# Bostanabad-Research-Group/GP-Plus

Hardware: AMD Instinct MI355X
Metric: MLL evals/sec (fwd+grad), NxN exact GP, N=20k d=8 (higher is better)
Workload: dtype f64; 1 GPU; C2: synthetic Borehole (Sobol seed 0, unique rows, z-scored) N=20000 d=8 fp64, GP_Plus Rough_RBF exact GP at theta1, one replica per GPU (restart-parallel); N=20000, d=8, streams_per_gpu=1

## Files before the change

gp-plus_amd/_lib.py:

```python
from __future__ import annotations

import ctypes
import os
import subprocess
from ctypes import POINTER, c_char_p, c_double, c_int, c_int32, c_int64, c_size_t, c_void_p
from pathlib import Path

import torch

_PKG_DIR = Path(__file__).resolve().parent
_LIB_PATH = _PKG_DIR / "libgpp_hip.so"
_CSRC = _PKG_DIR / "csrc"

_SIGNATURES = {
    "gpp_version": (c_char_p, []),
    "gpp_create": (c_int, [POINTER(c_void_p), c_int]),
    "gpp_destroy": (c_int, [c_void_p]),
    "gpp_set_stream": (c_int, [c_void_p, c_void_p]),
    "gpp_internal_stream": (c_int, [c_void_p, c_int, POINTER(c_void_p)]),
    "gpp_set_option": (c_int, [c_void_p, c_int, c_int]),
    "gpp_workspace_bytes": (c_size_t, [c_void_p, c_int, c_int64, c_int64, c_int, c_int]),
    "gpp_set_workspace": (c_int, [c_void_p, c_void_p, c_size_t]),
    "gpp_kernel_build": (c_int, [c_void_p, c_void_p, c_int64, c_int, c_void_p, c_void_p, c_void_p, c_void_p, c_int,
                                 c_double, c_int, c_int, c_int, c_void_p, c_int64, c_int64, c_int64]),
    "gpp_cross_kernel": (c_int, [c_void_p, c_void_p, c_int64, c_void_p, c_int64, c_int, c_void_p, c_void_p, c_int,
                                 c_int, c_void_p, c_int64]),
    "gpp_kernel_apply": (c_int, [c_void_p, c_void_p, c_int64, c_void_p, c_int64, c_int, c_void_p, c_void_p, c_int, c_int, c_void_p,
                                 c_int64, c_int, c_double, c_void_p, c_int64]),
    "gpp_rff_apply": (c_int, [c_void_p, c_void_p, c_int64, c_int, c_void_p, c_void_p, c_int64, c_void_p, c_void_p, c_int64, c_int,
                              c_double, c_void_p, c_int64]),
    "gpp_kernel_apply_grad": (c_int, [c_void_p, c_void_p, c_int64, c_void_p, c_int64, c_int, c_void_p, c_void_p, c_int, c_int, c_void_p,
                                      c_int64, c_int, c_void_p, c_int64, c_double, c_void_p, c_int64]),
    "gpp_rff_apply_grad": (c_int, [c_void_p, c_void_p, c_int64, c_int, c_void_p, c_void_p, c_int64, c_void_p, c_void_p, c_int64, c_int,
                                   c_void_p, c_int64, c_double, c_void_p, c_int64]),
    "gpp_potrf": (c_int, [c_void_p, c_void_p, c_int64, c_int64, c_void_p, c_int64, c_void_p]),
    "gpp_potrf_ws": (c_int, [c_void_p, c_void_p, c_int64, c_int64, c_void_p, c_int64, c_void_p, c_int64, c_void_p]),
    "gpp_build_potrf_ws": (c_int, [c_void_p, c_void_p, c_int64, c_int, c_void_p, c_void_p, c_void_p, c_void_p, c_int, c_double, c_int,
                                   c_int, c_void_p, c_int64, c_void_p, c_int64, c_void_p, c_int64, c_void_p]),
    "gpp_trtri": (c_int, [c_void_p, c_void_p, c_int64, c_int64, c_void_p, c_int64, c_void_p, c_int64]),
    "gpp_lauum": (c_int, [c_void_p, c_void_p, c_int64, c_int64, c_void_p, c_int64]),
    "gpp_lauum_grad": (c_int, [c_void_p, c_void_p, c_int64, c_int64, c_void_p, c_int, c_void_p, c_void_p, c_void_p, c_int, c_int, c_int,
                               c_void_p, c_void_p, c_void_p, c_void_p]),
    "gpp_post_cov_train": (c_int, [c_void_p, c_void_p, c_int64, c_int64, c_void_p, c_void_p, c_int, c_void_p, c_double, c_void_p,
                                   c_int64]),
    "gpp_syrk_rows": (c_int, [c_void_p, c_void_p, c_int64, c_void_p, c_int64, c_int64, c_int64, c_int64, c_int64, c_int, c_int]),
    "gpp_gemm_lower_cols": (c_int, [c_void_p, c_void_p, c_int64, c_void_p, c_int64, c_void_p, c_int64, c_int64, c_int64, c_double,
                                    c_double, c_int64, c_int64, c_int, c_int, c_int64, c_int64, c_int]),
    "gpp_shard_list_begin": (c_int, [c_void_p, c_int64, c_int64, c_int, c_int, c_void_p, c_int64, c_void_p, c_void_p, c_int64, c_void_p,
                                     c_void_p, c_void_p, c_void_p, c_int64, c_void_p, c_int, POINTER(c_int)]),
    "gpp_shard_piece_cols": (c_int64, []),
    "gpp_shard_list_gate": (c_int, [c_void_p, c_void_p, c_int, c_int]),
    "gpp_shard_list_signal": (c_int, [c_void_p, c_void_p, c_int, c_int]),
    "gpp_shard_list_end": (c_int, [c_void_p]),
    "gpp_set_comm": (c_int, [c_void_p, c_void_p, c_int, c_int]),
    "gpp_comm_unique_id": (c_int, [c_void_p]),
    "gpp_comm_init_rccl": (c_int, [c_void_p, c_void_p, c_int, c_int]),
    "gpp_shard_buffer_doubles": (c_size_t, [c_int64, c_int64, c_int, c_int, c_int]),
    "gpp_shard_eval": (c_int, [c_void_p, c_int64, c_int64, c_void_p, c_int, c_void_p, c_void_p, c_void_p, c_void_p, c_int, c_int, c_int,
                               c_double, c_int, c_int, c_void_p, POINTER(c_int)]),
    "gpp_push_create": (c_int, [c_int, c_int, c_int, c_int64, POINTER(c_void_p), c_void_p]),
    "gpp_push_connect": (c_int, [c_void_p, c_void_p]),
    "gpp_push_send": (c_int, [c_void_p, c_void_p, c_int64, c_void_p, c_int, c_int, POINTER(c_void_p), POINTER(c_int64), POINTER(c_int64),
                              POINTER(c_int64), POINTER(c_int64), POINTER(c_int64)]),
    "gpp_push_recv": (c_int, [c_void_p, c_void_p, c_int64, c_void_p, c_int, c_int, POINTER(c_void_p), POINTER(c_int64), POINTER(c_int64),
                              POINTER(c_int64), POINTER(c_int64), POINTER(c_int64)]),
    "gpp_push_ack": (c_int, [c_void_p, c_void_p, c_int64]),
    "gpp_push_info": (c_int, [c_void_p, POINTER(c_int64), POINTER(c_int)]),
    "gpp_push_destroy": (c_int, [c_void_p, c_int]),
    "gpp_shard_back_list": (c_int, [c_void_p, c_int64, c_int64, c_int, c_int, c_void_p, c_int64, c_void_p, c_void_p, c_int64, c_void_p,
                                    c_void_p, c_int, POINTER(c_int)]),
    "gpp_trmv_lower_cols": (c_int, [c_void_p, c_void_p, c_int64, c_int64, c_void_p, c_void_p, c_int64, c_int, c_int, c_int, c_int]),
    "gpp_mll_scalars": (c_int, [c_void_p, c_void_p, c_int64, c_int64, c_void_p, c_void_p]),
    "gpp_grad_reduce_cols": (c_int, [c_void_p, c_void_p, c_int64, c_int, c_void_p, c_void_p, c_void_p, c_int, c_int, c_int,
                                     c_void_p, c_void_p, c_int64, c_int, c_int64, c_int, c_int, c_void_p, c_void_p, c_void_p,
                                     c_void_p, c_int]),
    "gpp_lauum_rows": (c_int, [c_void_p, c_void_p, c_int64, c_int64, c_void_p, c_int64, c_int, c_int]),
    "gpp_lauum_rows_range": (c_int, [c_void_p, c_void_p, c_int64, c_int64, c_void_p, c_int64, c_int, c_int, c_int64, c_int64]),
    "gpp_transpose": (c_int, [c_void_p, c_void_p, c_int64, c_int64, c_int64, c_void_p, c_int64]),
    "gpp_mll_reduce": (c_int, [c_void_p, c_void_p, c_int64, c_void_p, c_int64, c_int64, c_void_p, c_void_p, c_void_p]),
    "gpp_alpha": (c_int, [c_void_p, c_void_p, c_int64, c_int64, c_void_p, c_void_p]),
    "gpp_grad_reduce": (c_int, [c_void_p, c_void_p, c_int64, c_int, c_void_p, c_void_p, c_void_p, c_int, c_int, c_int,
                                c_void_p, c_void_p, c_int64, c_int, c_void_p, c_void_p, c_void_p, c_void_p]),
    "gpp_loo_scalars": (c_int, [c_void_p, c_void_p, c_int64, c_int64, c_void_p, c_void_p, c_void_p, c_void_p, c_void_p, c_void_p, c_void_p,
                                c_void_p]),
    "gpp_sym_rowscale": (c_int, [c_void_p, c_void_p, c_int64, c_int64, c_void_p, c_void_p, c_int64]),
    "gpp_loo_grad_reduce": (c_int, [c_void_p, c_void_p, c_int64, c_int, c_void_p, c_void_p, c_void_p, c_int, c_int, c_int,
                                    c_void_p, c_void_p, c_void_p, c_int64, c_int, c_void_p, c_void_p, c_void_p, c_void_p]),
    "gpp_grad_reduce_rows": (c_int, [c_void_p, c_void_p, c_int64, c_int, c_void_p, c_void_p, c_void_p, c_int, c_int, c_int,
                                     c_void_p, c_void_p, c_int64, c_int, c_int64, c_int, c_int, c_void_p, c_void_p, c_void_p,
                                     c_void_p]),
    "gpp_predict": (c_int, [c_void_p, c_void_p, c_int64, c_int64, c_void_p, c_void_p, c_int64, c_int64, c_void_p,
                            c_void_p, c_int64, c_void_p, c_void_p]),
    "gpp_predict_tn": (c_int, [c_void_p, c_void_p, c_int64, c_int64, c_void_p, c_void_p, c_int64, c_int64, c_void_p,
                               c_void_p, c_int64, c_void_p, c_void_p]),
    "gpp_cross_grad": (c_int, [c_void_p, c_void_p, c_int64, c_void_p, c_int64, c_int, c_void_p, c_void_p, c_int, c_int, c_void_p,
                               c_void_p, c_void_p, c_void_p, c_int64, c_void_p, c_int, c_void_p, c_int, c_void_p, c_void_p]),
    "gpp_gemm": (c_int, [c_void_p, c_int, c_int, c_int64, c_int64, c_int64, c_double, c_void_p, c_int64, c_void_p,
                         c_int64, c_double, c_void_p, c_int64, c_int, c_int, c_int, c_int, c_int]),
    "gpp_gemm_batched": (c_int, [c_void_p, c_int, c_int, c_int64, c_int64, c_int64, c_double, c_void_p, c_int64, c_int64,
                                 c_void_p, c_int64, c_int64, c_double, c_void_p, c_int64, c_int64, c_int, c_int, c_int, c_int,
                                 c_int, c_int]),
    "gpp_kernel_build_batched": (c_int, [c_void_p, c_void_p, c_int64, c_int64, c_int, c_void_p, c_void_p, c_void_p, c_void_p, c_int,
                                         c_double, c_int, c_int, c_int, c_void_p, c_int64, c_int64, c_int]),
    "gpp_potrf_batched": (c_int, [c_void_p, c_void_p, c_int64, c_int64, c_int64, c_void_p, c_int64, c_int64, c_void_p, c_int]),
    "gpp_trtri_batched": (c_int, [c_void_p, c_void_p, c_int64, c_int64, c_int64, c_void_p, c_int64, c_int64, c_void_p, c_int64,
                                  c_int64, c_int]),
    "gpp_lauum_batched": (c_int, [c_void_p, c_void_p, c_int64, c_int64, c_int64, c_void_p, c_int64, c_int64, c_int]),
    "gpp_mll_reduce_batched": (c_int, [c_void_p, c_void_p, c_int64, c_int64, c_void_p, c_int64, c_int64, c_int64, c_void_p,
                                       c_void_p, c_int64, c_void_p, c_int]),
    "gpp_alpha_batched": (c_int, [c_void_p, c_void_p, c_int64, c_int64, c_int64, c_void_p, c_void_p, c_int64, c_int]),
    "gpp_grad_reduce_batched": (c_int, [c_void_p, c_void_p, c_int64, c_int64, c_int, c_void_p, c_void_p, c_void_p, c_int, c_int,
                                        c_int, c_void_p, c_int64, c_void_p, c_int64, c_int64, c_int, c_void_p, c_void_p, c_void_p,
                                        c_void_p, c_int]),
    "gpp_loo_scalars_batched": (c_int, [c_void_p, c_void_p, c_int64, c_int64, c_int64, c_void_p, c_void_p, c_void_p, c_void_p, c_void_p,
                                        c_void_p, c_void_p, c_int64, c_void_p, c_int]),
    "gpp_sym_rowscale_batched": (c_int, [c_void_p, c_void_p, c_int64, c_int64, c_int64, c_void_p, c_int64, c_void_p, c_int64, c_int64,
                                         c_int]),
    "gpp_loo_grad_reduce_batched": (c_int, [c_void_p, c_void_p, c_int64, c_int64, c_int, c_void_p, c_void_p, c_void_p, c_int, c_int,
                                            c_int, c_void_p, c_void_p, c_int64, c_void_p, c_int64, c_int64, c_int, c_void_p, c_void_p,
                                            c_void_p, c_void_p, c_int]),
    "gpp_cv_blocks": (c_int, [c_void_p, c_void_p, c_int64, c_int64, c_void_p, c_void_p, c_int, c_int, c_void_p, c_int64, c_int64]),
    "gpp_cv_rows": (c_int, [c_void_p, c_void_p, c_int64, c_int64, c_void_p, c_void_p, c_int, c_void_p, c_int64, c_int64, c_void_p,
                            c_int64]),
    "gpp_chol_append": (c_int, [c_void_p, c_void_p, c_int64, c_void_p, c_int64, c_int64, c_int64, c_void_p, c_int64, c_void_p, c_int64,
                                c_void_p, c_void_p, c_void_p, c_void_p]),
    "gpp_post_cross_sq": (c_int, [c_void_p, c_void_p, c_int64, c_void_p, c_int64, c_int, c_void_p, c_void_p, c_int, c_int, c_void_p,
                                  c_int64, c_void_p, c_int64, c_int64, c_int, c_void_p, c_void_p]),
    "gpp_post_cross_min": (c_int, [c_void_p, c_void_p, c_int64, c_void_p, c_int64, c_int, c_void_p, c_void_p, c_int, c_int, c_void_p,
                                   c_int64, c_void_p, c_int64, c_int64, c_int, c_void_p, c_void_p, c_void_p, c_int, c_void_p]),
    "gpp_cross_kernel_dx": (c_int, [c_void_p, c_void_p, c_int64, c_void_p, c_int64, c_int, c_void_p, c_void_p, c_int, c_int, c_int,
                                    c_int, c_void_p, c_int64]),
    "gpp_point_gram": (c_int, [c_void_p, c_void_p, c_int64, c_int64, c_int, c_int64, c_void_p, c_void_p, c_void_p]),
    "gpp_kernel_dxdx": (c_int, [c_void_p, c_void_p, c_int64, c_void_p, c_int64, c_int, c_void_p, c_void_p, c_int, c_int, c_int,
                                c_int, c_void_p, c_int64]),
}

_lib = None


class GppError(RuntimeError):
    """A libgpp_hip call returned a non-zero status."""


def build(force: bool = False) -> Path:
    if force:
        subprocess.run(["make", "-C", str(_CSRC), "clean"], check=True, capture_output=True)
    proc = subprocess.run(["make", "-C", str(_CSRC), "-j4"], capture_output=True, text=True)
    if proc.returncode != 0:
        raise RuntimeError("building libgpp_hip.so failed:\n" + proc.stdout + proc.stderr)
    return _LIB_PATH


def load() -> ctypes.CDLL:
    global _lib
    if _lib is not None:
        return _lib
    if not _LIB_PATH.exists():
        raise GppError(
            f"{_LIB_PATH} not found: the HIP extension is required (build it with "
            f"`make -C {_CSRC}` or `python -c 'import __graft_entry__ as g; g.build()'`); there is no CPU fallback."
        )
    lib = ctypes.CDLL(os.fspath(_LIB_PATH))
    for name, (restype, argtypes) in _SIGNATURES.items():
# ... 18 lines not shown
```

gp-plus_amd/backend.py:

```python
from __future__ import annotations

import atexit
import ctypes
import os
import threading
import weakref
from typing import Dict, Optional, Tuple

import torch

from . import _lib, settings
from ._lib import GppError, check

KIND_RBF, KIND_MATERN32, KIND_MATERN52 = 0, 1, 2
UPLO_FULL, UPLO_LOWER, UPLO_UPPER = 0, 1, 2
OPT_COOP_PANEL, OPT_PANEL_FAULT, OPT_PANEL_TIMEOUT_MS, OPT_EXEC_SCHED, OPT_DAG_SCHED = 1, 2, 3, 4, 5
OPT_GEMM_TILE = 6
OP_MLL_EVAL, OP_PREDICT, OP_PREDICT_GRAD = 0, 1, 2
OP_APPLY = 3
OP_APPLY_GRAD = 4
OP_APPEND = 5
OP_POST_CROSS = 6
OP_POST_CROSS_MIN = 7
OP_POINT_GRAM = 8
# ... 208 lines not shown
    @_on_own_device
    def kernel_apply(self, Ua, Ub, w, sf2, C, out, *, beta=0.0, kind=KIND_RBF, d_split=0):
        M, D, N, S = self._apply_checks(Ua, Ub, C, out, sf2)
        _need(w, torch.float64, "w")
        if w.numel() != D:
            raise GppError(f"w has {w.numel()} entries for {D} features")
        self._stream()
        check(self.lib.gpp_kernel_apply(self.h, Ua.data_ptr(), M, Ub.data_ptr(), N, D, w.data_ptr(), sf2.data_ptr(), kind, d_split,
                                        C.data_ptr(), _ld(C), S, float(beta), out.data_ptr(), _ld(out)), "gpp_kernel_apply")
        return out

    @_on_own_device
    def rff_apply(self, Ua, omega, phase, sf2, theta, out, *, beta=0.0):
        M, D, F, S = self._apply_checks(Ua, omega, theta, out, sf2)
        _need(phase, torch.float64, "phase")
        if phase.numel() != F:
            raise GppError(f"phase has {phase.numel()} entries for {F} features")
        self._stream()
        check(self.lib.gpp_rff_apply(self.h, Ua.data_ptr(), M, D, omega.data_ptr(), phase.data_ptr(), F, sf2.data_ptr(),
                                     theta.data_ptr(), _ld(theta), S, float(beta), out.data_ptr(), _ld(out)), "gpp_rff_apply")
        return out

    @_on_own_device
    def kernel_apply_grad(self, Ua, Ub, w, sf2, C, gbar, g_Ua, *, beta=0.0, kind=KIND_RBF, d_split=0):
        M, D, N, S = self._apply_checks(Ua, Ub, C, gbar, sf2, g_Ua)
        _need(w, torch.float64, "w")
        if w.numel() != D:
            raise GppError(f"w has {w.numel()} entries for {D} features")
        self._stream()
        check(self.lib.gpp_kernel_apply_grad(self.h, Ua.data_ptr(), M, Ub.data_ptr(), N, D, w.data_ptr(), sf2.data_ptr(), kind, d_split,
                                             C.data_ptr(), _ld(C), S, gbar.data_ptr(), _ld(gbar), float(beta), g_Ua.data_ptr(),
                                             _ld(g_Ua)), "gpp_kernel_apply_grad")
        return g_Ua

    @_on_own_device
    def rff_apply_grad(self, Ua, omega, phase, sf2, theta, gbar, g_Ua, *, beta=0.0):
        M, D, F, S = self._apply_checks(Ua, omega, theta, gbar, sf2, g_Ua)
        _need(phase, torch.float64, "phase")
        if phase.numel() != F:
            raise GppError(f"phase has {phase.numel()} entries for {F} features")
        self._stream()
        check(self.lib.gpp_rff_apply_grad(self.h, Ua.data_ptr(), M, D, omega.data_ptr(), phase.data_ptr(), F, sf2.data_ptr(),
                                          theta.data_ptr(), _ld(theta), S, gbar.data_ptr(), _ld(gbar), float(beta), g_Ua.data_ptr(),
                                          _ld(g_Ua)), "gpp_rff_apply_grad")
        return g_Ua

    @_on_own_device
    def potrf(self, A, Linv, info, T=None):
        _need(A, torch.float64, "A"); _need(Linv, torch.float64, "Linv"); _need(info, torch.int32, "info")
        self._stream()
        if T is None:
            check(self.lib.gpp_potrf(self.h, A.data_ptr(), A.shape[0], _ld(A), Linv.data_ptr(), _ld(Linv), info.data_ptr()),
                  "gpp_potrf")
        else:
            check(self.lib.gpp_potrf_ws(self.h, A.data_ptr(), A.shape[0], _ld(A), Linv.data_ptr(), _ld(Linv), T.data_ptr(),
                                        _ld(T), info.data_ptr()), "gpp_potrf_ws")

    @_on_own_device
    def build_potrf(self, U, w, sf2, tau, grp, A, Linv, info, T, *, jitter=0.0, kind=KIND_RBF, d_split=0):
        N, D = U.shape
        _check_features(D)
        for t, n in ((U, "U"), (w, "w"), (sf2, "sf2"), (A, "A"), (Linv, "Linv"), (T, "T")):
            _need(t, torch.float64, n)
        _need(info, torch.int32, "info")
        if tau is not None:
            _need(tau, torch.float64, "tau")
        S = 0 if tau is None else tau.numel()
        if grp is not None:
            self._check_groups(grp, N, S)
        if not U.is_contiguous():
            raise GppError("U must be contiguous")
        self._stream()
        check(self.lib.gpp_build_potrf_ws(self.h, U.data_ptr(), N, D, w.data_ptr(), sf2.data_ptr(), _ptr(tau), _ptr(grp), S,
                                          float(jitter), kind, d_split, A.data_ptr(), _ld(A), Linv.data_ptr(), _ld(Linv),
                                          T.data_ptr(), _ld(T), info.data_ptr()), "gpp_build_potrf_ws")

    @_on_own_device
    def trtri(self, U, Linv, T):
        self._stream()
        check(self.lib.gpp_trtri(self.h, U.data_ptr(), U.shape[0], _ld(U), Linv.data_ptr(), _ld(Linv), T.data_ptr(), _ld(T)),
              "gpp_trtri")

    @_on_own_device
    def lauum(self, Linv, Kinv):
        self._stream()
        check(self.lib.gpp_lauum(self.h, Linv.data_ptr(), Linv.shape[0], _ld(Linv), Kinv.data_ptr(), _ld(Kinv)), "gpp_lauum")

    @_on_own_device
    def lauum_grad(self, Linv, U, w, sf2, grp, S, alpha, dU, g_w, g_sf2, g_tau, *, kind=KIND_RBF) -> bool:
        N, D = U.shape
        for t, n in ((Linv, "Linv"), (U, "U"), (w, "w"), (sf2, "sf2"), (alpha, "alpha"), (g_w, "g_w"), (g_sf2, "g_sf2"),
                     (g_tau, "g_tau")):
            _need(t, torch.float64, n)
        if grp is not None:
            self._check_groups(grp, N, S)
        if not U.is_contiguous():
            raise GppError("U must be contiguous")
        self.ensure_workspace(OP_MLL_EVAL, N, 0, D, S)
        self._stream()
        status = self.lib.gpp_lauum_grad(self.h, Linv.data_ptr(), N, _ld(Linv), U.data_ptr(), D, w.data_ptr(), sf2.data_ptr(),
                                         _ptr(grp), S, kind, dU, alpha.data_ptr(), g_w.data_ptr(), g_sf2.data_ptr(),
                                         g_tau.data_ptr())
        if status == NOT_SUPPORTED:
            return False
        if status == NO_WORKSPACE:
            raise GppError("gpp_lauum_grad: the handle's scratch workspace is missing or too small")
        check(status, "gpp_lauum_grad")
        return True

    @_on_own_device
    def post_cov_train(self, Kinv, tau, grp, d, out, *, jitter=0.0):
        N = Kinv.shape[0]
        for t, n in ((Kinv, "Kinv"), (tau, "tau"), (out, "A")):
            _need(t, torch.float64, n)
        if d is not None:
            _need(d, torch.float64, "d")
            if d.numel() != N or not d.is_contiguous():
                raise GppError(f"d must be a contiguous vector of {N} doubles")
        if grp is not None:
            self._check_groups(grp, N, tau.numel())
        if out.shape[0] != N or out.shape[1] != N:
            raise GppError("post_cov_train: shapes do not match")
        self._stream()
        check(self.lib.gpp_post_cov_train(self.h, Kinv.data_ptr(), N, _ld(Kinv), tau.data_ptr(), _ptr(grp), tau.numel(), _ptr(d),
                                          float(jitter), out.data_ptr(), _ld(out)), "gpp_post_cov_train")
        return out

    @_on_own_device
    def syrk_rows(self, Urow, C, nb, first_block, rank, nranks):
        self._stream()
        check(self.lib.gpp_syrk_rows(self.h, Urow.data_ptr(), _ld(Urow), C.data_ptr(), _ld(C), C.shape[0], Urow.shape[0], nb,
                                     first_block, rank, nranks), "gpp_syrk_rows")

    @_on_own_device
    def shard_list_begin(self, N, nb, rank, nranks, A, Kc, Lc, D, W, info, workers=0) -> bool:
        self._stream()
        used = ctypes.c_int(0)
        check(self.lib.gpp_shard_list_begin(self.h, N, nb, rank, nranks, A.data_ptr(), _ld(A), Kc.data_ptr(), Lc.data_ptr(), _ld(Kc),
                                            D.data_ptr(), W[0].data_ptr(), W[1].data_ptr(), W[2].data_ptr(), _ld(W[0]),
                                            info.data_ptr(), int(workers), ctypes.byref(used)), "gpp_shard_list_begin")
        return bool(used.value)

    def shard_messages(self, N: int, nb: int, k: int):
        o, o2 = k * nb, min((k + 2) * nb, N)
        W = int(self.lib.gpp_shard_piece_cols()) or N
        return [(o, o2)] + [(c, min(c + W, N)) for c in range(o2, N, W)]

    @_on_own_device
    def shard_list_gate(self, stream, tail: int, k: int) -> None:
        check(self.lib.gpp_shard_list_gate(self.h, ctypes.c_void_p(stream.cuda_stream), int(tail), k), "gpp_shard_list_gate")

    @_on_own_device
    def shard_list_signal(self, stream, tail: int, k: int) -> None:
        check(self.lib.gpp_shard_list_signal(self.h, ctypes.c_void_p(stream.cuda_stream), int(tail), k), "gpp_shard_list_signal")

    @_on_own_device
    def shard_list_end(self) -> None:
        self._stream()
        check(self.lib.gpp_shard_list_end(self.h), "gpp_shard_list_end")

    @_on_own_device
    def shard_back_list(self, N, nb, rank, nranks, A, Kc, Lc, D, info, workers=0) -> bool:
        self._stream()
        used = ctypes.c_int(0)
        check(self.lib.gpp_shard_back_list(self.h, N, nb, rank, nranks, A.data_ptr(), _ld(A), Kc.data_ptr(), Lc.data_ptr(), _ld(Kc),
                                           D.data_ptr(), info.data_ptr(), int(workers), ctypes.byref(used)), "gpp_shard_back_list")
        return bool(used.value)

    @_on_own_device
    def gemm_lower_cols(self, A, B, C, alpha, beta, nb, first_block, rank, nranks, row0=0, row1=None, compact=False):
        M, K = A.shape[1], A.shape[0]
        if compact:
            if B.shape[0] != K or C.shape[0] != M:
                raise GppError("gemm_lower_cols: shapes do not match")
        elif A.shape != B.shape or C.shape[0] != C.shape[1] or C.shape[0] != M:
            raise GppError("gemm_lower_cols: shapes do not match")
        self._stream()
        check(self.lib.gpp_gemm_lower_cols(self.h, A.data_ptr(), _ld(A), B.data_ptr(), _ld(B), C.data_ptr(), _ld(C), M,
                                           K, float(alpha), float(beta), nb, first_block, rank, nranks, row0,
                                           M if row1 is None else row1, 1 if compact else 0),
              "gpp_gemm_lower_cols")

    @_on_own_device
    def trmv_lower_cols(self, T, x, y, nb, rank, nranks, trans=False, compact=False):
        for t, n in ((x, "x"), (y, "y")):
            _need(t, torch.float64, n)
        if trans:
            self.ensure_workspace(OP_MLL_EVAL, T.shape[0], 0, 1, 1)
        self._stream()
        check(self.lib.gpp_trmv_lower_cols(self.h, T.data_ptr(), _ld(T), T.shape[0], x.data_ptr(), y.data_ptr(), nb, rank, nranks,
                                           1 if trans else 0, 1 if compact else 0), "gpp_trmv_lower_cols")

    @_on_own_device
    def mll_scalars(self, U, z, out3):
        self._stream()
        check(self.lib.gpp_mll_scalars(self.h, U.data_ptr(), _ld(U), U.shape[0], z.data_ptr(), out3.data_ptr()), "gpp_mll_scalars")

    @_on_own_device
    def lauum_rows(self, Linv, Kinv, rank, nranks):
        self._stream()
        check(self.lib.gpp_lauum_rows(self.h, Linv.data_ptr(), Linv.shape[0], _ld(Linv), Kinv.data_ptr(), _ld(Kinv), rank, nranks),
              "gpp_lauum_rows")

    @_on_own_device
    def lauum_rows_range(self, Linv, Kinv, rank, nranks, row0, row1):
        self._stream()
        check(self.lib.gpp_lauum_rows_range(self.h, Linv.data_ptr(), Linv.shape[0], _ld(Linv), Kinv.data_ptr(), _ld(Kinv), rank,
                                            nranks, row0, row1), "gpp_lauum_rows_range")

    @_on_own_device
    def transpose(self, src, dst):
        if src.shape[0] != dst.shape[1] or src.shape[1] != dst.shape[0]:
            raise GppError("transpose: shapes do not match")
        self._stream()
        check(self.lib.gpp_transpose(self.h, src.data_ptr(), src.stride(0), src.shape[0], src.shape[1], dst.data_ptr(), dst.stride(0)),
              "gpp_transpose")

    @_on_own_device
    def mll_reduce(self, L, Linv, r, z, out3):
        for t, n in ((r, "r"), (z, "z"), (out3, "out3")):
            _need(t, torch.float64, n)
        self._stream()
        check(self.lib.gpp_mll_reduce(self.h, L.data_ptr(), _ld(L), Linv.data_ptr(), _ld(Linv), L.shape[0], r.data_ptr(),
                                      z.data_ptr(), out3.data_ptr()), "gpp_mll_reduce")

    @_on_own_device
    def alpha(self, Linv, z, alpha):
        N = Linv.shape[0]
        self._stream()
        check(self.lib.gpp_alpha(self.h, Linv.data_ptr(), _ld(Linv), N, z.data_ptr(), alpha.data_ptr()), "gpp_alpha")

    @_on_own_device
    def grad_reduce(self, U, w, sf2, grp, S, alpha, Kinv, dU, g_w, g_sf2, g_tau, g_U, *, kind=KIND_RBF, d_split=0):
        N, D = U.shape
        if grp is not None:
            self._check_groups(grp, N, S)
        self.ensure_workspace(OP_MLL_EVAL, N, 0, D, S)
        self._stream()
        check(self.lib.gpp_grad_reduce(self.h, U.data_ptr(), N, D, w.data_ptr(), sf2.data_ptr(), _ptr(grp), S, kind,
                                       d_split, alpha.data_ptr(), Kinv.data_ptr(), _ld(Kinv), dU, g_w.data_ptr(),
                                       g_sf2.data_ptr(), g_tau.data_ptr(), _ptr(g_U)), "gpp_grad_reduce")

    @_on_own_device
    def loo_scalars(self, Linv, alpha, y, d, mu=None, s2=None, a=None, sqrtb=None, loo=None):
        N = Linv.shape[0]
        _need(Linv, torch.float64, "Linv")
        for t, n, size in ((alpha, "alpha", N), (y, "y", N), (d, "d", N), (mu, "mu", N), (s2, "s2", N), (a, "a", N),
                           (sqrtb, "sqrtb", N), (loo, "loo", 1)):
            if t is None:
                continue
            _need(t, torch.float64, n)
            if t.numel() < size or not t.is_contiguous():
                raise GppError(f"{n} must be a contiguous vector of {size} doubles")
        if mu is not None and y is None:
            raise GppError("loo_scalars: mu needs y")
        self._stream()
        check(self.lib.gpp_loo_scalars(self.h, Linv.data_ptr(), _ld(Linv), N, alpha.data_ptr(), _ptr(y), d.data_ptr(), _ptr(mu),
                                       _ptr(s2), _ptr(a), _ptr(sqrtb), _ptr(loo)), "gpp_loo_scalars")

    @_on_own_device
    def sym_rowscale(self, Kinv, s, out):
        N = Kinv.shape[0]
        for t, n in ((Kinv, "Kinv"), (s, "s"), (out, "S")):
            _need(t, torch.float64, n)
        if out.shape[0] != N or out.shape[1] != N or s.numel() != N or not s.is_contiguous():
            raise GppError("sym_rowscale: shapes do not match")
        if out.data_ptr() == Kinv.data_ptr():
            raise GppError("sym_rowscale works out of place")
        self._stream()
        check(self.lib.gpp_sym_rowscale(self.h, Kinv.data_ptr(), N, _ld(Kinv), s.data_ptr(), out.data_ptr(), _ld(out)),
              "gpp_sym_rowscale")
        return out

    @_on_own_device
    def loo_grad_reduce(self, U, w, sf2, grp, S, alpha, beta, C, dU, g_w, g_sf2, g_tau, g_U, *, kind=KIND_RBF, d_split=0):
        N, D = U.shape
        _check_features(D)
        for t, n in ((alpha, "alpha"), (beta, "beta")):
            _need(t, torch.float64, n)
            if t.numel() != N or not t.is_contiguous():
                raise GppError(f"{n} must be a contiguous vector of {N} doubles")
        if grp is not None:
            self._check_groups(grp, N, S)
        self.ensure_workspace(OP_MLL_EVAL, N, 0, D, S)
        self._stream()
        check(self.lib.gpp_loo_grad_reduce(self.h, U.data_ptr(), N, D, w.data_ptr(), sf2.data_ptr(), _ptr(grp), S, kind, d_split,
                                           alpha.data_ptr(), beta.data_ptr(), C.data_ptr(), _ld(C), dU, g_w.data_ptr(),
                                           g_sf2.data_ptr(), g_tau.data_ptr(), _ptr(g_U)), "gpp_loo_grad_reduce")

    @_on_own_device
    def grad_reduce_rows(self, U, w, sf2, grp, S, alpha, Kinv, dU, nb, rank, nranks, g_w, g_sf2, g_tau, g_U, *,
                         kind=KIND_RBF, d_split=0):
        N, D = U.shape
        if grp is not None:
            self._check_groups(grp, N, S)
        self.ensure_workspace(OP_MLL_EVAL, N, 0, D, S)
        self._stream()
        check(self.lib.gpp_grad_reduce_rows(self.h, U.data_ptr(), N, D, w.data_ptr(), sf2.data_ptr(), _ptr(grp), S, kind,
                                            d_split, alpha.data_ptr(), Kinv.data_ptr(), _ld(Kinv), dU, nb, rank, nranks,
                                            g_w.data_ptr(), g_sf2.data_ptr(), g_tau.data_ptr(), _ptr(g_U)),
              "gpp_grad_reduce_rows")

    @_on_own_device
    def grad_reduce_cols(self, U, w, sf2, grp, S, alpha, Kinv, dU, nb, rank, nranks, g_w, g_sf2, g_tau, g_U, *,
                         kind=KIND_RBF, d_split=0, compact=False):
        N, D = U.shape
        if grp is not None:
# ... 512 lines not shown
```

gp-plus_amd/csrc/gpp_api.hip:

```cpp
#include "../../include/gpp.h"
#include "gpp_internal.h"

#include <algorithm>
#include <cmath>
#include <cstdio>
#include <cstdlib>
#include <cstring>
#include <new>

const GppEnv& gpp_env() {
  static const GppEnv env = [] {
    auto num = [](const char* name, long long unset) { const char* v = getenv(name); return v ? atoll(v) : unset; };
    GppEnv e;
    e.coop_panel = num("GPP_COOP_PANEL", 1) != 0;
    e.dag_sched = num("GPP_DAG_SCHED", 1) != 0;
    e.dag_phased = num("GPP_DAG_PHASED", 0) != 0;
    e.shard_list = num("GPP_SHARD_LIST", 1) != 0;
    e.shard_workers = (int)num("GPP_SHARD_WORKERS", 0);
    e.shard_fill = (int)num("GPP_SHARD_FILL", -1);
    e.shard_timeout_ms = num("GPP_SHARD_TIMEOUT_MS", 60000);
    const int64_t cols = num("GPP_SHARD_PIECE_COLS", 8192);
    e.shard_piece_cols = cols <= 0 ? (int64_t)0 : std::max<int64_t>(GPP_TILE, cols / GPP_TILE * GPP_TILE);
    e.sharded_force_collectives = num("GPP_SHARDED_FORCE_COLLECTIVES", 0) != 0;
    e.exec_verbose = getenv("GPP_EXEC_VERBOSE") != nullptr;
// ... 67 lines not shown
    if (e != hipSuccess) return e;
    if (rem == 0) break;
    double* Bp = c.A + oo * c.ld + (oo + nb);
    GemmArgs g = mk(c.Li + oo * c.ldi + oo, c.ldi, Bp, c.ld, Bp, c.ld, nb, rem, nb, 1.0, 0.0);
    g.a_mask = 1;
    e = gpp_launch_gemm(c.s, 2, g, 1, NBLK, 32);
    if (e != hipSuccess) return e;
    GemmArgs u = mk(Bp, c.ld, Bp, c.ld, c.A + (oo + nb) * c.ld + (oo + nb), c.ld, rem, rem, nb, -1.0, 1.0);
    u.c_lower = 2;
    e = gpp_launch_gemm(c.s, 2, u, 1, 32, 32);
    if (e != hipSuccess) return e;
  }
  return hipSuccess;
}

hipError_t potrf_blk_batched(const Ctx& c, int64_t n, int batch, int64_t sA, int64_t sLi) {
  for (int64_t j0 = 0; j0 < n; j0 += NBLK) {
    const int64_t nb = std::min<int64_t>(NBLK, n - j0), oo = j0, rem = n - j0 - nb;
    hipError_t e = gpp_launch_leaf(c.s, c.A + oo * c.ld + oo, c.ld, c.Li + oo * c.ldi + oo, c.ldi, (int)nb, c.info, (int)oo,
                                   batch, sA, sLi);
    if (e != hipSuccess) return e;
    if (rem == 0) break;
    double* Bp = c.A + oo * c.ld + (oo + nb);
    GemmArgs g = mk(c.Li + oo * c.ldi + oo, c.ldi, Bp, c.ld, Bp, c.ld, nb, rem, nb, 1.0, 0.0);
    g.a_mask = 1;
    g.sA = sLi; g.sB = sA; g.sC = sA;
    e = gpp_launch_gemm(c.s, 2, g, batch, NBLK, 32);
    if (e != hipSuccess) return e;
    GemmArgs u = mk(Bp, c.ld, Bp, c.ld, c.A + (oo + nb) * c.ld + (oo + nb), c.ld, rem, rem, nb, -1.0, 1.0);
    u.c_lower = 2;
    u.sA = sA; u.sB = sA; u.sC = sA;
    e = gpp_launch_gemm(c.s, 2, u, batch, 32, 32);
    if (e != hipSuccess) return e;
  }
  return hipSuccess;
}

hipError_t potrf_rec(const Ctx& c, int64_t o, int64_t n) {
  if (n <= 0) return hipSuccess;
  if (n <= NBLK)
    return gpp_launch_leaf(c.s, c.A + o * c.ld + o, c.ld, c.Li + o * c.ldi + o, c.ldi, (int)n, c.info, (int)o);
  if (n <= BLK_MAX) return potrf_blk(c, o, n);
  const int64_t n1 = split(n), n2 = n - n1;
  hipError_t e = potrf_rec(c, o, n1);
  if (e != hipSuccess) return e;
  e = trsm_rec(c, o + n1, n2, o, n1);
  if (e != hipSuccess) return e;
  const double* U12 = c.A + o * c.ld + (o + n1);
  GemmArgs g = mk(U12, c.ld, U12, c.ld, c.A + (o + n1) * c.ld + (o + n1), c.ld, n2, n2, n1, -1.0, 1.0);
  g.c_lower = 2;
  e = gpp_launch_gemm(c.s, 2, g, 1);
  if (e != hipSuccess) return e;
  return potrf_rec(c, o + n1, n2);
}

constexpr int64_t PANEL_MAX_N = 2048;
inline bool panel_fits(const gpp_handle_s* h, int64_t n) {
  return h->coop_panel && h->panel_flags && h->ncu >= 2 && n > 2 * NBLK && n <= PANEL_MAX_N && (n + NBLK - 1) / NBLK <= gpp_panel_max_leaves();
}
hipError_t launch_panel_at(gpp_handle_s* h, const Ctx& c, int64_t o, int64_t n, int max_wgs) {
  if (h->panel_fault) {
    h->panel_fault = 0;
    return gpp_launch_fill_i32(c.s, c.info, 1, GPP_INFO_PANEL_TIMEOUT);
  }
  hipStreamCaptureStatus cap = hipStreamCaptureStatusNone;
  if (hipStreamIsCapturing(c.s, &cap) != hipSuccess) {
    (void)hipGetLastError();
    cap = hipStreamCaptureStatusNone;
  }
  int slot;
  if (cap == hipStreamCaptureStatusActive) slot = GPP_PANEL_RING + (h->cap_next++ % GPP_PANEL_CAP_RING);
  else slot = h->panel_next++ % GPP_PANEL_RING;
  int* fl = reinterpret_cast<int*>(h->panel_flags + (size_t)slot * gpp_panel_flag_bytes());
  return gpp_launch_panel(c.s, c.A, c.ld, c.Li, c.ldi, (int)n, c.info, (int)o, fl, max_wgs, h->panel_timeout_ms);
}

hipError_t launch_panel(gpp_handle_s* h, const Ctx& c, int64_t o, int64_t n, int max_wgs) {
  Ctx b = c;
  b.A = c.A + o * c.ld + o;
  b.Li = c.Li + o * c.ldi + o;
  return launch_panel_at(h, b, o, n, max_wgs);
}

template <typename Skip>
hipError_t trtri_level(hipStream_t st, const double* U, int64_t ld, double* Linv, int64_t ldi, double* T, int64_t ldt,
                       int64_t base, int64_t n, int64_t s, Skip skip, int mbatch = 1, int64_t msU = 0, int64_t msLi = 0,
                       int64_t msT = 0, int g1_tile = 0, hipEvent_t before_g2 = nullptr) {
  const int64_t npairs_full = n / (2 * s);
  const int64_t rem = n - npairs_full * 2 * s;
  auto launch = [&](int64_t o, int64_t m2, int batch) -> hipError_t {
    const int64_t pstride_U = 2 * s * (ld + 1), pstride_I = 2 * s * (ldi + 1), pstride_T = 2 * s * (ldt + 1);
    GemmArgs g1 = mk(U + o * ld + (o + s), ld, Linv + o * ldi + o, ldi, T + (o + s) * ldt + o, ldt, m2, s, s, 1.0, 0.0);
    g1.b_mask = 2; g1.klo_mode = 2; g1.col_major = 1;
    g1.sA = pstride_U; g1.sB = pstride_I; g1.sC = pstride_T;
    g1.batch2 = mbatch; g1.zA = msU; g1.zB = msLi; g1.zC = msT;
    g1.batch_fast = 1;
    hipError_t e = gpp_launch_gemm(st, 2, g1, batch, g1_tile, g1_tile);
    if (e != hipSuccess) return e;
    if (before_g2) {
      e = hipStreamWaitEvent(st, before_g2, 0);
      if (e != hipSuccess) return e;
    }
    GemmArgs g2 = mk(Linv + (o + s) * ldi + (o + s), ldi, T + (o + s) * ldt + o, ldt, Linv + (o + s) * ldi + o, ldi, m2, s,
                     m2, -1.0, 0.0);
    g2.a_mask = 1; g2.khi_mode = 1; g2.row_reverse = 1;
    g2.sA = pstride_I; g2.sB = pstride_T; g2.sC = pstride_I;
    g2.C2 = Linv + o * ldi + (o + s); g2.ldc2 = ldi; g2.sC2 = pstride_I;
    g2.batch2 = mbatch; g2.zA = msLi; g2.zB = msT; g2.zC = msLi; g2.zC2 = msLi;
    g2.batch_fast = 1;
    return gpp_launch_gemm(st, 2, g2, batch);
  };
  int64_t p = 0;
  while (p < npairs_full) {
    if (skip(base + 2 * s * p)) { ++p; continue; }
    int64_t q = p;
    while (q < npairs_full && !skip(base + 2 * s * q)) ++q;
    hipError_t e = launch(base + 2 * s * p, s, (int)(q - p));
    if (e != hipSuccess) return e;
    p = q;
  }
  if (rem > s && !skip(base + npairs_full * 2 * s)) {
    hipError_t e = launch(base + npairs_full * 2 * s, rem - s, 1);
    if (e != hipSuccess) return e;
  }
  return hipSuccess;
}

constexpr int PANEL_CUS = 32;
constexpr int64_t BORDER_MAX_N = 11264;
constexpr int64_t BORDER_MIN_N = 3840;
constexpr int64_t BORDER_FULL_MIN_N = 9216;
constexpr int64_t SPLIT_ELEMS = 30000000;
hipError_t ensure_streams(gpp_handle_s* h) {
  if (h->cu_split < 0) {
    hipDeviceProp_t prop;
    hipError_t e = hipGetDeviceProperties(&prop, h->device);
    if (e != hipSuccess) return e;
    const int ncu = prop.multiProcessorCount;
    h->cu_split = 0;
    if (ncu >= 4 * PANEL_CUS && ncu <= 1024) {
      uint32_t mp[32] = {0}, mu[32] = {0};
      const int words = (ncu + 31) / 32;
      for (int c = 0; c < ncu; ++c) (c < PANEL_CUS ? mp : mu)[c >> 5] |= 1u << (c & 31);
      hipStream_t sp = nullptr, su = nullptr, sf = nullptr;
      if (hipExtStreamCreateWithCUMask(&sp, words, mp) == hipSuccess &&
          hipExtStreamCreateWithCUMask(&su, words, mu) == hipSuccess &&
          hipExtStreamCreateWithCUMask(&sf, words, mu) == hipSuccess) {
        h->panel_stream = sp;
        h->upd_stream = su;
        h->fill_stream = sf;
        h->cu_split = 1;
        h->panel_cus = PANEL_CUS;
      } else {
        (void)hipGetLastError();
        if (sp) (void)hipStreamDestroy(sp);
        if (su) (void)hipStreamDestroy(su);
        if (sf) (void)hipStreamDestroy(sf);
      }
    }
    if (!h->cu_split) {
      static bool warned = false;
      if (!warned) {
        warned = true;
        fprintf(stderr, "libgpp_hip: hipExtStreamCreateWithCUMask unavailable on device %d (%d CUs): the look-ahead factorisation "
                        "falls back to priority streams and will be markedly slower\n", h->device, ncu);
      }
      int lo = 0, hi = 0;
      e = hipDeviceGetStreamPriorityRange(&lo, &hi);
      if (e != hipSuccess) return e;
      e = hipStreamCreateWithPriority(&h->panel_stream, hipStreamNonBlocking, hi);
      if (e != hipSuccess) return e;
      e = hipStreamCreateWithFlags(&h->upd_stream, hipStreamNonBlocking);
      if (e != hipSuccess) return e;
      e = hipStreamCreateWithFlags(&h->fill_stream, hipStreamNonBlocking);
      if (e != hipSuccess) return e;
    }
  }
  if (!h->full_stream) {
    hipError_t e = hipStreamCreateWithFlags(&h->full_stream, hipStreamNonBlocking);
    if (e != hipSuccess) return e;
  }
  while (h->n_events < 16) {
    hipError_t e = hipEventCreateWithFlags(&h->events[h->n_events], hipEventDisableTiming);
    if (e != hipSuccess) return e;
    ++h->n_events;
  }
  return hipSuccess;
}
inline hipEvent_t next_event(gpp_handle_s* h) {
  hipEvent_t ev = h->events[h->ev_next];
  h->ev_next = (h->ev_next + 1) % 16;
  return ev;
}
#define HIP_TRY(expr)                \
  do {                               \
    hipError_t _e = (expr);          \
    if (_e != hipSuccess) return _e; \
  } while (0)

hipError_t potrf_lookahead(gpp_handle_s* h, const Ctx& cm, int64_t N, int64_t NB, double* T, int64_t ldt) {
  HIP_TRY(ensure_streams(h));
  Ctx cp = cm, cu = cm;
  cp.s = h->panel_stream;
  cu.s = h->upd_stream;
  hipEvent_t ev = next_event(h);
// ... 356 lines not shown
  DagPlan* P = nullptr;
  if (h)
    for (int i = 0; i < GPP_DAG_PLANS; ++i)
      if (h->dag_plans[i] && (!P || h->dag_plans[i]->stamp > P->stamp)) P = h->dag_plans[i];
  return P;
}
int gpp_debug_split_builds(gpp_handle_t h) { return h ? h->split_builds : -1; }
int gpp_debug_dag_info(gpp_handle_t h, int64_t* info8) {
  const DagPlan* P = dag_mru(h);
  if (!P) return -1;
  info8[8] = P->inv_rows;
  info8[9] = P->N;
  info8[0] = (int64_t)P->tasks.size(); info8[1] = (int64_t)P->groups.size(); info8[2] = P->B; info8[3] = P->nt;
  info8[4] = P->ncounters; info8[5] = (int64_t)(P->sim_ms * 1000.0); info8[6] = (int64_t)(P->sim_busy * 1000.0); info8[7] = P->flags;
  return 0;
}
int gpp_debug_dag_counters(gpp_handle_t h, int* out, int nmax) {
  DagPlan* P = dag_mru(h);
  if (!P || !P->d_counters) return -1;
  if (hipDeviceSynchronize() != hipSuccess) return 1;
  std::vector<int> c(P->ncounters);
  if (hipMemcpy(c.data(), P->d_counters, c.size() * sizeof(int), hipMemcpyDeviceToHost) != hipSuccess) return 2;
  int n = 0;
  auto put = [&](int v) { if (n < nmax) out[n++] = v; };
  put(c[0]); put(c[1]); put(P->B);
  for (int b = 0; b < P->B; ++b) put(c[P->c_pd + b]);
  for (int b = 0; b < P->B; ++b) put(c[P->c_g1d + b]);
  if (P->flags & DAG_SHARD) {
    for (int b = 0; b < P->B; ++b) put(c[P->c_cph + b]);
    for (int b = 0; b < P->B; ++b) put(c[P->c_cpt + b * P->GP]);
    for (int b = 0; b < P->B; ++b) put(c[P->c_art + b * P->GP]);
  }
  return n;
}
int gpp_debug_dag_trace(gpp_handle_t h, int on) {
  DagPlan* P = dag_mru(h);
  if (!P) return -1;
  if (hipDeviceSynchronize() != hipSuccess) return 1;
  if (on && !P->d_trace) {
    if (hipMalloc(&P->d_trace, 4 * P->tasks.size() * sizeof(unsigned long long)) != hipSuccess) return 2;
    (void)hipMemset(P->d_trace, 0, 4 * P->tasks.size() * sizeof(unsigned long long));
  } else if (!on && P->d_trace) {
    (void)hipFree(P->d_trace);
    P->d_trace = nullptr;
  }
  return 0;
}
int gpp_debug_dag_fetch(gpp_handle_t h, void* tasks, void* trace) {
  const DagPlan* P = dag_mru(h);
  if (!P) return -1;
  if (hipDeviceSynchronize() != hipSuccess) return 1;
  if (tasks) memcpy(tasks, P->tasks.data(), P->tasks.size() * sizeof(DagTask));
  if (trace) {
    if (!P->d_trace) return 2;
    if (hipMemcpy(trace, P->d_trace, 4 * P->tasks.size() * sizeof(unsigned long long), hipMemcpyDeviceToHost) != hipSuccess) return 3;
  }
  return 0;
}

int gpp_create(gpp_handle_t* out, int device) {
  if (!out) return -1;
  int ndev = 0;
  hipError_t e = hipGetDeviceCount(&ndev);
  if (e != hipSuccess) return rc(e);
  if (device < 0 || device >= ndev) return -2;
  e = hipSetDevice(device);
  if (e != hipSuccess) return rc(e);
  gpp_handle_s* h = new (std::nothrow) gpp_handle_s();
  if (!h) return rc(hipErrorOutOfMemory);
  h->device = device;
  h->stream = nullptr;
  h->ws = nullptr;
  h->ws_bytes = 0;
  h->panel_stream = nullptr;
  h->upd_stream = nullptr;
  h->fill_stream = nullptr;
  h->full_stream = nullptr;
  h->cu_split = -1;
  h->panel_cus = 0;
  h->n_events = 0;
  h->ev_next = 0;
  h->inv_N = 0;
  h->inv_nblocks = 0;
  h->panel_flags = nullptr;
  h->panel_next = 0;
  h->coop_panel = gpp_env().coop_panel ? 1 : 0;
  h->panel_fault = 0;
  h->panel_timeout_ms = 500;
  for (int i = 0; i < GPP_DAG_PLANS; ++i) h->dag_plans[i] = nullptr;
  h->shard_cur = nullptr;
  h->shard_info = nullptr;
  h->shard_ready = nullptr;
  h->dag_clock = 0;
  h->dag_sched = 1;
  h->gemm_tile = 0;
  h->ncu = 0;
  if (hipDeviceGetAttribute(&h->ncu, hipDeviceAttributeMultiprocessorCount, device) != hipSuccess || h->ncu < 2) {
    (void)hipGetLastError();
    h->ncu = 0;
  }
  h->cap_next = 0;
  h->handoff = nullptr;
  if (hipMalloc(reinterpret_cast<void**>(&h->panel_flags), (GPP_PANEL_RING + GPP_PANEL_CAP_RING) * gpp_panel_flag_bytes()) != hipSuccess ||
      hipMemset(h->panel_flags, 0, (GPP_PANEL_RING + GPP_PANEL_CAP_RING) * gpp_panel_flag_bytes()) != hipSuccess) {
    (void)hipGetLastError();
    if (h->panel_flags) (void)hipFree(h->panel_flags);
    h->panel_flags = nullptr;
  }
  *out = h;
  return 0;
}

int gpp_destroy(gpp_handle_t h) {
  if (!h) return -1;
  for (hipStream_t s : {h->panel_stream, h->upd_stream, h->fill_stream, h->full_stream})
    if (s) (void)hipStreamSynchronize(s);
  if (h->full_stream) (void)hipStreamDestroy(h->full_stream);
  if (h->fill_stream) (void)hipStreamDestroy(h->fill_stream);
  if (h->upd_stream) (void)hipStreamDestroy(h->upd_stream);
  if (h->panel_stream) (void)hipStreamDestroy(h->panel_stream);
  for (int i = 0; i < h->n_events; ++i) (void)hipEventDestroy(h->events[i]);
  if (h->handoff) (void)hipEventDestroy(h->handoff);
  if (h->shard_ready) (void)hipEventDestroy(h->shard_ready);
  if (h->panel_flags) (void)hipFree(h->panel_flags);
  for (int i = 0; i < GPP_DAG_PLANS; ++i)
    if (h->dag_plans[i]) gpp_dag_free(h->dag_plans[i]);
  gpp_shard_release_comm(h);
  delete h;
  return 0;
}

int gpp_set_stream(gpp_handle_t h, void* stream) {
  if (!h) return -1;
  hipStream_t s = reinterpret_cast<hipStream_t>(stream);
  if (s != h->stream) {
    hipStreamCaptureStatus a = hipStreamCaptureStatusNone, b = hipStreamCaptureStatusNone;
    if (hipStreamIsCapturing(h->stream, &a) != hipSuccess || hipStreamIsCapturing(s, &b) != hipSuccess) {
      (void)hipGetLastError();
      a = b = hipStreamCaptureStatusActive;
    }
    auto internal = [&](hipStream_t q) { return q && (q == h->panel_stream || q == h->upd_stream || q == h->fill_stream || q == h->full_stream); };
    if (a == hipStreamCaptureStatusNone && b == hipStreamCaptureStatusNone && !internal(s) && !internal(h->stream)) {
      if (!h->handoff) GPP_TRY(hipEventCreateWithFlags(&h->handoff, hipEventDisableTiming));
      GPP_TRY(hipEventRecord(h->handoff, h->stream));
      GPP_TRY(hipStreamWaitEvent(s, h->handoff, 0));
    }
    h->stream = s;
  }
  return 0;
}

int gpp_set_option(gpp_handle_t h, int option, int value) {
  if (!h) return -1;
  if (option == GPP_OPT_COOP_PANEL) h->coop_panel = value ? 1 : 0;
  else if (option == GPP_OPT_PANEL_FAULT) h->panel_fault = value ? 1 : 0;
  else if (option == GPP_OPT_DAG_SCHED || option == GPP_OPT_EXEC_SCHED) h->dag_sched = value ? 1 : 0;
  else if (option == GPP_OPT_PANEL_TIMEOUT_MS) {
    if (value < 1 || value > 60000) return -3;
    h->panel_timeout_ms = value;
  } else if (option == GPP_OPT_GEMM_TILE) {
    if (value < 0 || value > 4) return -3;
    h->gemm_tile = value;
  } else return -2;
  return 0;
}

// ... 129 lines not shown
  if (target > 0) GPP_TRY(gpp_launch_exec_gate(s, P->d_counters, tail ? P->c_cpt + piece : P->c_cph + k, target, h->shard_info, budget));
  return 0;
}

int gpp_shard_list_signal(gpp_handle_t h, void* stream, int tail, int k) {
  if (!h || !h->shard_cur) return -1;
  const DagPlan* P = h->shard_cur;
  if (k < 0 || k >= P->B || k % P->nranks == P->rank) return -4;
  if (tail < 0 || tail > shard_pieces(P, k)) return -3;
  GPP_TRY(hipStreamWaitEvent(reinterpret_cast<hipStream_t>(stream), h->shard_ready, 0));
  return rc(gpp_launch_exec_signal(reinterpret_cast<hipStream_t>(stream), P->d_counters, tail ? P->c_art + k * P->GP + tail - 1 : P->c_pd + k));
}

int gpp_shard_list_end(gpp_handle_t h) {
  if (!h || !h->shard_cur) return -1;
  DagPlan* P = h->shard_cur;
  h->shard_cur = nullptr;
  hipEvent_t E = next_event(h), F = next_event(h);
  GPP_TRY(hipEventRecord(E, h->upd_stream));
  GPP_TRY(hipEventRecord(F, h->panel_stream));
  GPP_TRY(hipStreamWaitEvent(h->stream, E, 0));
  GPP_TRY(hipStreamWaitEvent(h->stream, F, 0));
  GPP_TRY(hipEventRecord(P->last_use, h->stream));
  return 0;
}

int gpp_shard_back_list(gpp_handle_t h, int64_t N, int64_t nb, int rank, int nranks, const double* A, int64_t ld, double* Kc, double* Lc,
                        int64_t ldc, const double* D, int32_t* info, int workers, int* used) {
  if (!h) return -1;
  if (!used) return -14;
  *used = 0;
  if (N < 2 || nb < 128 || nb % 128 != 0) return -2;
  if (rank < 0 || nranks < 1 || rank >= nranks) return -4;
  if (int e = check_mat(A, ld, N, 6)) return e;
  if (!Kc || !aligned16(Kc)) return -8;
  if (!Lc || !aligned16(Lc)) return -9;
  const int64_t wc = ((N + nb - 1) / nb - rank + nranks - 1) / nranks * nb;
  if ((ldc & 1) || ldc < wc) return -10;
  if (!D || !aligned16(D)) return -11;
  if (!info) return -12;
  const GppEnv& env = gpp_env();
  if (!env.shard_list || !h->dag_sched || N < SHARD_LIST_MIN_N || N > DAG_MAX_N || h->shard_cur) return 0;
  if (workers <= 0 && env.shard_workers > 0) workers = 2 * env.shard_workers;
  GPP_TRY(ensure_streams(h));
  const int flags = DAG_SHARD | DAG_BACK;
  const int nworkers = workers > 0 ? workers : 2 * h->ncu;
  DagPlan* P = dag_plan_cached(h, PlanKey{N, nb, ld, ldc, ld, flags, 0, rank, nranks, workers}, [&]() -> DagPlan* {
    DagTuning tune = gpp_dag_default_tuning();
    tune.workers = nworkers;
    tune.fill = 0;
    tune.inv_rows = 0;
    tune.fuse = dag_fuse(N);
    DagPlan* Q = gpp_dag_plan(N, nb, ld, ldc, ld, 0, flags, tune, rank, nranks);
    if (!Q) return nullptr;
    Q->workers = workers;
    if (Q->tasks.empty() || gpp_dag_upload(Q) != hipSuccess) {
      (void)hipGetLastError();
      gpp_dag_free(Q);
      return nullptr;
    }
    return Q;
  });
  if (!P) return 0;
  hipStream_t sm = h->stream;
  GPP_TRY(gpp_launch_fill_i32(sm, P->d_counters, P->ncounters, 0));
  DagBases bases{{const_cast<char*>(reinterpret_cast<const char*>(A)), reinterpret_cast<char*>(Kc), reinterpret_cast<char*>(Lc),
                  const_cast<char*>(reinterpret_cast<const char*>(D)), nullptr, nullptr, nullptr, nullptr}};
  GPP_TRY(gpp_launch_dag_bind(sm, P->d_groups, P->d_groups_abs, (int)P->groups.size(), bases));
  DagLaunch dl{};
  dl.groups = P->d_groups_abs; dl.tasks = P->d_tasks; dl.ntasks = (int)P->tasks.size();
  dl.counters = P->d_counters; dl.info = info;
  dl.budget = shard_budget(h);
  dl.max_tasks = 0; dl.quit_id = -1; dl.quit_val = 0; dl.ticket_limit = 0;
  dl.trace = P->d_trace; dl.tag = 0;
  GPP_TRY(gpp_launch_dag(sm, nworkers, dl));
  GPP_TRY(hipEventRecord(P->last_use, sm));
  *used = 1;
  return 0;
}

size_t gpp_workspace_bytes(gpp_handle_t h, int op, int64_t N, int64_t M, int D, int S) {
  (void)h;
  if (op == GPP_OP_MLL_EVAL) {
    return std::max({gpp_grad_ws_bytes(N, D, S, D), gpp_trmv_t_ws_bytes(N), gpp_lauum_grad_ws_bytes(N, D)}) + 256;
  }
  if (op == GPP_OP_PREDICT) return 256;
  if (op == GPP_OP_PREDICT_GRAD) return gpp_pgrad_ws_bytes(M, N, D, D, S) + 256;
  if (op == GPP_OP_APPLY) return gpp_apply_ws_bytes(N, M, S) + 256;
  if (op == GPP_OP_APPLY_GRAD) return gpp_apply_ws_bytes(N, M, D) + 256;
  if (op == GPP_OP_APPEND) return gpp_append_ws_bytes(N, M) + 256;
  if (op == GPP_OP_POST_CROSS) return gpp_post_cross_ws_bytes(M, N) + 256;
  if (op == GPP_OP_POST_CROSS_MIN) return gpp_post_cross_min_ws_bytes(M, N, S) + 256;
  if (op == GPP_OP_POINT_GRAM) return gpp_point_gram_ws_bytes(M, D) + 256;
  return 0;
}

int gpp_set_workspace(gpp_handle_t h, void* ws, size_t bytes) {
  if (!h) return -1;
  if (ws && !aligned16(ws)) return -2;
  h->ws = ws;
  h->ws_bytes = bytes;
  return 0;
}

int gpp_kernel_build(gpp_handle_t h, const double* U, int64_t N, int D, const double* w, const double* sf2,
                     const double* tau, const int32_t* grp, int S, double jitter, int kind, int d_split, int uplo,
                     double* Ky, int64_t ld, int64_t row0, int64_t nrows) {
  if (!h) return -1;
  if (!U) return -2;
  if (N < 0) return -3;
  if (D < 1 || D > 64) return -4;
  if (!w) return -5;
  if (!sf2) return -6;
  if (tau && S < 1) return -9;
  if (kind < 0 || kind > 2) return -11;
  if (d_split < 0 || d_split > D) return -12;
  if (uplo != GPP_UPLO_FULL && uplo != GPP_UPLO_LOWER && uplo != GPP_UPLO_UPPER) return -13;
  if (!Ky) return -14;
  if (ld < N) return -15;
  if (row0 < 0 || nrows < 0 || row0 + nrows > N || (row0 % 64) != 0) return -16;
  if (uplo == GPP_UPLO_UPPER && (row0 != 0 || nrows != N)) return -16;
  GPP_TRY(gpp_launch_kernel_build(h->stream, U, N, D, w, sf2, tau, grp, S, jitter, kind, d_split, uplo, Ky, ld, row0, nrows));
  return 0;
}

int gpp_cross_kernel(gpp_handle_t h, const double* Ua, int64_t Ma, const double* Ub, int64_t Nb, int D, const double* w,
                     const double* sf2, int kind, int d_split, double* Kab, int64_t ld) {
  if (!h) return -1;
  if (!Ua) return -2;
  if (Ma < 0) return -3;
  if (!Ub) return -4;
  if (Nb < 0) return -5;
  if (D < 1 || D > 64) return -6;
  if (!w) return -7;
  if (!sf2) return -8;
  if (kind < 0 || kind > 2) return -9;
  if (d_split < 0 || d_split > D) return -10;
  if (!Kab) return -11;
  if (ld < Nb) return -12;
  GPP_TRY(gpp_launch_cross_kernel(h->stream, Ua, Ma, Ub, Nb, D, w, sf2, kind, d_split, Kab, ld));
  return 0;
}

int gpp_kernel_apply(gpp_handle_t h, const double* Ua, int64_t M, const double* Ub, int64_t N, int D, const double* w,
                     const double* sf2, int kind, int d_split, const double* C, int64_t ldc, int S, double beta, double* Out,
                     int64_t ldo) {
  if (!h) return -1;
  if (!Ua) return -2;
  if (M < 1) return -3;
  if (!Ub) return -4;
  if (N < 1) return -5;
  if (D < 1 || D > 64) return -6;
  if (!w) return -7;
  if (!sf2) return -8;
  if (kind < 0 || kind > 2) return -9;
  if (d_split < 0 || d_split > D) return -10;
  if (!C) return -11;
  if (S < 1) return -13;
  if (ldc < S) return -12;
  if (!Out) return -15;
  if (ldo < S) return -16;
  if (gpp_apply_pieces(N) > 1 && (!h->ws || h->ws_bytes < gpp_apply_ws_bytes(N, M, S))) return GPP_NO_WORKSPACE;
  GPP_TRY(gpp_launch_kernel_apply(h->stream, Ua, M, Ub, N, D, w, sf2, kind, d_split, C, ldc, S, beta, Out, ldo, h->ws, h->ws_bytes));
  return 0;
}

int gpp_rff_apply(gpp_handle_t h, const double* Ua, int64_t M, int D, const double* Omega, const double* phase, int64_t F,
// ... 69 lines not shown
static int potrf_ws_impl(gpp_handle_t h, double* A, int64_t N, int64_t ld, double* Linv, int64_t ldi, double* T, int64_t ldt,
                         int32_t* info_dev, const KyBuild* build) {
  if (!h) return -1;
  if (N < 0) return -3;
  if (int r = check_mat(A, ld, N, 2)) return r;
  if (int r = check_mat(Linv, ldi, N, 5)) return r;
  if (T) {
    if (int r = check_mat(T, ldt, N, 7)) return r;
  }
  if (!info_dev) return -9;
  GPP_TRY(gpp_launch_fill_i32(h->stream, info_dev, 1, 0));
  Ctx c{h->stream, A, ld, Linv, ldi, info_dev};
  h->inv_N = N;
  h->inv_nblocks = 0;
  const int64_t la_min = T ? BORDER_MIN_N : 6 * LOOKAHEAD_NB;
  bool dag_used = false;
  hipStreamCaptureStatus cap = hipStreamCaptureStatusNone;
  if (build) GPP_TRY(hipStreamIsCapturing(h->stream, &cap));
  if (build && cap != hipStreamCaptureStatusNone) {
    GPP_TRY((*build)(h->stream, c, N, 0, N));
    build = nullptr;
  }
  GPP_TRY(potrf_dag(h, c, N, T, ldt, &dag_used, build));
  if (dag_used) return 0;
  if (build) GPP_TRY((*build)(h->stream, c, N, 0, N));
  if (N >= la_min) {
    GPP_TRY(potrf_lookahead(h, c, N, LOOKAHEAD_NB, T, ldt));
  } else if (panel_fits(h, N)) {
    int wgs = h->ncu;
    if (h->cu_split == 1 && h->stream == h->panel_stream) wgs = h->panel_cus;
    else if (h->cu_split == 1 && (h->stream == h->upd_stream || h->stream == h->fill_stream)) wgs = h->ncu - h->panel_cus;
    else if (h->stream) {
      uint32_t mask[32] = {0};
      if (hipExtStreamGetCUMask(h->stream, 32, mask) == hipSuccess) {
        int cus = 0;
        for (int c = 0; c < h->ncu && c < 1024; ++c) cus += (mask[c >> 5] >> (c & 31)) & 1u;
        if (cus >= 2 && cus < wgs) wgs = cus;
      } else {
        (void)hipGetLastError();
      }
    }
    GPP_TRY(launch_panel(h, c, 0, N, wgs));
    h->inv_nblocks = 1;
    h->inv_o[0] = 0;
    h->inv_n[0] = N;
  } else {
    GPP_TRY(potrf_rec(c, 0, N));
  }
  return 0;
}

int gpp_potrf_ws(gpp_handle_t h, double* A, int64_t N, int64_t ld, double* Linv, int64_t ldi, double* T, int64_t ldt,
                 int32_t* info_dev) {
  return potrf_ws_impl(h, A, N, ld, Linv, ldi, T, ldt, info_dev, nullptr);
}

int gpp_build_potrf_ws(gpp_handle_t h, const double* U, int64_t N, int D, const double* w, const double* sf2, const double* tau,
                       const int32_t* grp, int S, double jitter, int kind, int d_split, double* A, int64_t ld, double* Linv,
                       int64_t ldi, double* T, int64_t ldt, int32_t* info_dev) {
  if (!h) return -1;
  if (!U) return -2;
  if (N < 0) return -3;
  if (D < 1 || D > 64) return -4;
  if (!w) return -5;
  if (!sf2) return -6;
  if (tau && S < 1) return -9;
  if (kind < 0 || kind > 2) return -11;
  if (d_split < 0 || d_split > D) return -12;
  if (int r = check_mat(A, ld, N, 13)) return r;
  if (int r = check_mat(Linv, ldi, N, 15)) return r;
  if (T) {
    if (int r = check_mat(T, ldt, N, 17)) return r;
  }
  if (!info_dev) return -19;
  const KyBuild build{U, w, sf2, tau, grp, D, S, kind, d_split, jitter};
  return potrf_ws_impl(h, A, N, ld, Linv, ldi, T, ldt, info_dev, &build);
}

int gpp_potrf(gpp_handle_t h, double* A, int64_t N, int64_t ld, double* Linv, int64_t ldi, int32_t* info_dev) {
  const int r = gpp_potrf_ws(h, A, N, ld, Linv, ldi, nullptr, 0, info_dev);
  return r == -9 ? -7 : r;
}

int gpp_trtri(gpp_handle_t h, const double* U, int64_t N, int64_t ld, double* Linv, int64_t ldi, double* T, int64_t ldt) {
  if (!h) return -1;
  if (N < 0) return -3;
  if (int r = check_mat(U, ld, N, 2)) return r;
  if (int r = check_mat(Linv, ldi, N, 5)) return r;
  if (int r = check_mat(T, ldt, N, 7)) return r;
  const bool have = (h->inv_N == N && h->inv_nblocks > 0);
  for (int64_t s = NBLK; s < N; s *= 2) {
    auto skip = [&](int64_t b) {
      if (!have) return false;
      for (int i = 0; i < h->inv_nblocks; ++i)
        if (b >= h->inv_o[i] && b + 2 * s <= h->inv_o[i] + h->inv_n[i]) return true;
      for (int i = 0; i < h->inv_nblocks; ++i)
        if (b >= h->inv_o[i] && h->inv_o[i] + h->inv_n[i] == N && b + s < N) return true;
      return false;
    };
    GPP_TRY(trtri_level(h->stream, U, ld, Linv, ldi, T, ldt, 0, N, s, skip));
  }
  h->inv_N = 0;
  return 0;
}

int gpp_lauum(gpp_handle_t h, const double* Linv, int64_t N, int64_t ldi, double* Kinv, int64_t ldk) {
  if (!h) return -1;
  if (N < 0) return -3;
  if (int r = check_mat(Linv, ldi, N, 2)) return r;
  if (int r = check_mat(Kinv, ldk, N, 5)) return r;
  GemmArgs g = mk(Linv, ldi, Linv, ldi, Kinv, ldk, N, N, N, 1.0, 0.0);
  g.a_mask = 2; g.b_mask = 2; g.klo_mode = 3; g.c_lower = 1; g.tag = 1;
  const int t = N <= 2560 ? 32 : N <= 5120 ? 64 : NBLK;
  GPP_TRY(gpp_launch_gemm(h->stream, 2, g, 1, t, t));
  return 0;
}

int gpp_lauum_grad(gpp_handle_t h, const double* Linv, int64_t N, int64_t ldi, const double* U, int D, const double* w,
                   const double* sf2, const int32_t* grp, int S, int kind, int dU, const double* alpha, double* g_w,
                   double* g_sf2, double* g_tau) {
  if (!h) return -1;
  if (N < 0) return -3;
  if (int r = check_mat(Linv, ldi, N, 2)) return r;
  if (!U) return -5;
  if (D < 1 || D > 64) return -6;
  if (!w) return -7;
  if (!sf2) return -8;
  if (S < 1 || S > 64) return -10;
  if (kind < 0 || kind > 2) return -11;
  if (dU < 0 || dU > D) return -12;
  if (!alpha) return -13;
  if (!g_w) return -14;
  if (!g_sf2) return -15;
  if (!g_tau) return -16;
  if (kind != GPP_KIND_RBF || D > 16 || dU != 0) return GPP_NOT_SUPPORTED;
  if (!h->ws || h->ws_bytes < gpp_lauum_grad_ws_bytes(N, D)) return GPP_NO_WORKSPACE;
  GemmArgs g = mk(Linv, ldi, Linv, ldi, nullptr, ldi, N, N, N, 1.0, 0.0);
  g.a_mask = 2; g.b_mask = 2; g.klo_mode = 3; g.c_lower = 1;
  const int64_t tiles = (N + NBLK - 1) / NBLK, nrec = tiles * (tiles + 1) / 2;
  double* rec = reinterpret_cast<double*>(h->ws);
  double* wdiag = rec + nrec * (D + 1);
  GPP_TRY(gpp_launch_lauum_grad(h->stream, g, GradEpiArgs{U, w, sf2, alpha, rec, wdiag, D}));
  GPP_TRY(gpp_launch_grad_finish(h->stream, rec, nrec, D, S, wdiag, grp, N, g_w, g_sf2, g_tau));
  return 0;
}

int gpp_post_cov_train(gpp_handle_t h, const double* Kinv, int64_t N, int64_t ldk, const double* tau, const int32_t* grp, int S,
                       const double* d, double jitter, double* A, int64_t lda) {
  if (!h) return -1;
  if (N < 0) return -3;
  if (int r = check_mat(Kinv, ldk, N, 2)) return r;
  if (!tau) return -5;
  if (S < 1) return -7;
  if (int r = check_mat(A, lda, N, 10)) return r;
  if (A == Kinv && lda != ldk) return -11;
  GPP_TRY(gpp_launch_post_cov_train(h->stream, Kinv, ldk, N, tau, grp, d, jitter, A, lda));
  return 0;
}

int gpp_lauum_rows(gpp_handle_t h, const double* Linv, int64_t N, int64_t ldi, double* Kinv, int64_t ldk, int rank, int nranks) {
  if (!h) return -1;
  if (N < 0) return -3;
  if (int r = check_mat(Linv, ldi, N, 2)) return r;
  if (int r = check_mat(Kinv, ldk, N, 5)) return r;
  if (nranks < 1 || rank < 0 || rank >= nranks) return -7;
  GemmArgs g = mk(Linv, ldi, Linv, ldi, Kinv, ldk, N, N, N, 1.0, 0.0);
  g.a_mask = 2; g.b_mask = 2; g.klo_mode = 3; g.c_lower = 1; g.tag = 1;
  g.row_mod = nranks; g.row_off = rank;
  GPP_TRY(gpp_launch_gemm(h->stream, 2, g, 1, NBLK, NBLK));
  return 0;
}

int gpp_lauum_rows_range(gpp_handle_t h, const double* Linv, int64_t N, int64_t ldi, double* Kinv, int64_t ldk, int rank,
                         int nranks, int64_t row0, int64_t row1) {
  if (!h) return -1;
  if (N < 0) return -3;
  if (int r = check_mat(Linv, ldi, N, 2)) return r;
  if (int r = check_mat(Kinv, ldk, N, 5)) return r;
  if (nranks < 1 || rank < 0 || rank >= nranks) return -7;
  if (row0 < 0 || row1 < row0 || row1 > N || (row0 % NBLK) != 0) return -9;
  if (row1 == row0) return 0;
  GemmArgs g = mk(Linv, ldi, Linv, ldi, Kinv, ldk, N, N, N, 1.0, 0.0);
  g.a_mask = 2; g.b_mask = 2; g.klo_mode = 3; g.c_lower = 1; g.tag = 1;
  g.row_mod = nranks; g.row_off = rank;
  const int64_t t0 = row0 / NBLK, t1 = (row1 + NBLK - 1) / NBLK;
// ... 15 lines not shown
}

int gpp_syrk_rows(gpp_handle_t h, const double* Urow, int64_t ldu, double* C, int64_t ldc, int64_t Nt, int64_t K, int64_t nb,
                  int64_t first_block, int rank, int nranks) {
  if (!h) return -1;
  if (!Urow || !aligned16(Urow) || (ldu & 1)) return -2;
  if (!C || !aligned16(C) || (ldc & 1)) return -4;
  if (Nt < 0 || K < 0) return -6;
  if (nb < NBLK || nb % NBLK != 0) return -8;
  if (first_block < 0) return -9;
  if (nranks < 1 || rank < 0 || rank >= nranks) return -10;
  if (Nt == 0 || K == 0) return 0;
  GemmArgs g = mk(Urow, ldu, Urow, ldu, C, ldc, Nt, Nt, K, -1.0, 1.0);
  g.c_lower = 2;
  g.own_mod = nranks;
  g.own_bt = (int)(nb / NBLK);
  g.own_off = (int)(((first_block - rank) % nranks + nranks) % nranks);
  GPP_TRY(gpp_launch_gemm(h->stream, 2, g, 1, NBLK, NBLK));
  return 0;
}

int gpp_gemm_lower_cols(gpp_handle_t h, const double* A, int64_t lda, const double* B, int64_t ldb, double* C, int64_t ldc,
                        int64_t M, int64_t K, double alpha, double beta, int64_t nb, int64_t first_block, int rank, int nranks,
                        int64_t row0, int64_t row1, int compact) {
  if (!h) return -1;
  if (!A || !aligned16(A) || (lda & 1)) return -2;
  if (!B || !aligned16(B) || (ldb & 1)) return -4;
  if (!C || !aligned16(C) || (ldc & 1)) return -6;
  if (M < 0 || K < 0) return -8;
  if (nb < NBLK || nb % NBLK != 0) return -12;
  if (first_block < 0) return -13;
  if (nranks < 1 || rank < 0 || rank >= nranks) return -14;
  if (row0 < 0 || row1 < row0 || row1 > M || row0 % NBLK != 0) return -16;
  if (M == 0 || K == 0 || row1 == row0) return 0;
  GemmArgs g = mk(A, lda, B, ldb, C, ldc, M, M, K, alpha, beta);
  g.c_lower = 1;
  g.row_t0 = (int)(row0 / NBLK);
  g.row_t1 = (int)((row1 + NBLK - 1) / NBLK);
  g.own_mod = nranks;
  g.own_bt = (int)(nb / NBLK);
  g.own_off = (int)(((first_block - rank) % nranks + nranks) % nranks);
  g.compact_bc = compact ? 1 : 0;
  GPP_TRY(gpp_launch_gemm(h->stream, 2, g, 1, NBLK, NBLK));
  return 0;
}

int gpp_trmv_lower_cols(gpp_handle_t h, const double* T, int64_t ldt, int64_t N, const double* x, double* y, int64_t nb, int rank,
                        int nranks, int trans, int compact) {
  if (!h) return -1;
  if (N < 0) return -4;
  if (int q = check_mat(T, ldt, compact ? std::min<int64_t>(N, ldt) : N, 2)) return q;
  if (!x || !aligned16(x)) return -5;
  if (!y) return -6;
  if (nb < 64 || nb % 64 != 0) return -7;
  if (nranks < 1 || rank < 0 || rank >= nranks) return -8;
  if (trans != 0 && trans != 1) return -10;
  if (trans && (!h->ws || h->ws_bytes < gpp_trmv_t_ws_bytes(N))) return -1;
  if (compact && nranks >= 1 && rank >= 0 && ldt < owned_cols(N, nb, rank, nranks)) return -3;
  GPP_TRY(gpp_launch_trmv_lower_cols(h->stream, T, ldt, N, x, y, nb, rank, nranks, trans, h->ws, h->ws_bytes, compact));
  return 0;
}

int gpp_mll_scalars(gpp_handle_t h, const double* U, int64_t ld, int64_t N, const double* z, double* out3) {
  if (!h) return -1;
  if (N < 0) return -4;
  if (int q = check_mat(U, ld, N, 2)) return q;
  if (!z) return -5;
  if (!out3) return -6;
  GPP_TRY(gpp_launch_mll_scalars(h->stream, U, ld, N, z, out3));
  return 0;
}

int gpp_mll_reduce(gpp_handle_t h, const double* U, int64_t ld, const double* Linv, int64_t ldi, int64_t N,
                   const double* r, double* z, double* out3) {
  if (!h) return -1;
  if (N < 0) return -6;
  if (int q = check_mat(U, ld, N, 2)) return q;
  if (int q = check_mat(Linv, ldi, N, 4)) return q;
  if (!r || !aligned16(r)) return -7;
  if (!z) return -8;
  if (!out3) return -9;
  GPP_TRY(gpp_launch_trmv_lower(h->stream, Linv, ldi, N, r, z));
  GPP_TRY(gpp_launch_mll_scalars(h->stream, U, ld, N, z, out3));
  return 0;
}

int gpp_alpha(gpp_handle_t h, const double* Linv, int64_t ldi, int64_t N, const double* z, double* alpha) {
  if (!h) return -1;
  if (N < 0) return -4;
  if (int q = check_mat(Linv, ldi, N, 2)) return q;
  if (!z || !aligned16(z)) return -5;
  if (!alpha) return -6;
  GPP_TRY(gpp_launch_trmv_upper(h->stream, Linv, ldi, N, z, alpha));
  return 0;
}

int gpp_grad_reduce(gpp_handle_t h, const double* U, int64_t N, int D, const double* w, const double* sf2,
                    const int32_t* grp, int S, int kind, int d_split, const double* alpha, const double* Kinv,
                    int64_t ldk, int dU, double* g_w, double* g_sf2, double* g_tau, double* g_U) {
  if (!h) return -1;
  if (!U) return -2;
  if (N < 0) return -3;
  if (D < 1 || D > 64) return -4;
  if (!w) return -5;
  if (!sf2) return -6;
  if (S < 1 || S > 64) return -8;
  if (kind < 0 || kind > 2) return -9;
  if (d_split < 0 || d_split > D) return -10;
  if (!alpha) return -11;
  if (int q = check_mat(Kinv, ldk, N, 12)) return q;
  if (dU < 0 || dU > D) return -14;
  if (!g_w) return -15;
  if (!g_sf2) return -16;
  if (!g_tau) return -17;
  if (dU > 0 && !g_U) return -18;
  if (!h->ws || h->ws_bytes < gpp_grad_ws_bytes(N, D, S, dU)) return -1;
  GPP_TRY(gpp_launch_grad_reduce(h->stream, U, N, D, w, sf2, grp, S, kind, d_split, alpha, Kinv, ldk, dU, g_w, g_sf2, g_tau,
                                 g_U, h->ws, h->ws_bytes));
  return 0;
}

int gpp_loo_scalars(gpp_handle_t h, const double* Linv, int64_t ldi, int64_t N, const double* alpha, const double* y, double* d,
                    double* mu, double* s2, double* a, double* sqrtb, double* loo) {
  if (!h) return -1;
  if (N < 0) return -4;
  if (int q = check_mat(Linv, ldi, N, 2)) return q;
  if (!alpha) return -5;
  if (mu && !y) return -6;
  if (!d) return -7;
  GPP_TRY(gpp_launch_loo_scalars(h->stream, Linv, ldi, N, alpha, y, d, mu, s2, a, sqrtb, loo));
  return 0;
}

int gpp_sym_rowscale(gpp_handle_t h, const double* Kinv, int64_t N, int64_t ldk, const double* s, double* S, int64_t lds) {
  if (!h) return -1;
  if (N < 0) return -3;
  if (int r = check_mat(Kinv, ldk, N, 2)) return r;
  if (!s) return -5;
  if (int r = check_mat(S, lds, N, 6)) return r;
  if (S == Kinv) return -6;
  GPP_TRY(gpp_launch_sym_rowscale(h->stream, Kinv, ldk, N, s, S, lds));
  return 0;
}

int gpp_loo_grad_reduce(gpp_handle_t h, const double* U, int64_t N, int D, const double* w, const double* sf2,
                        const int32_t* grp, int S, int kind, int d_split, const double* alpha, const double* beta,
                        const double* C, int64_t ldc, int dU, double* g_w, double* g_sf2, double* g_tau, double* g_U) {
  if (!h) return -1;
  if (!U) return -2;
  if (N < 0) return -3;
  if (D < 1 || D > 64) return -4;
  if (!w) return -5;
  if (!sf2) return -6;
  if (S < 1 || S > 64) return -8;
  if (kind < 0 || kind > 2) return -9;
  if (d_split < 0 || d_split > D) return -10;
  if (!alpha) return -11;
  if (!beta) return -12;
  if (int q = check_mat(C, ldc, N, 13)) return q;
  if (dU < 0 || dU > D) return -15;
  if (!g_w) return -16;
  if (!g_sf2) return -17;
  if (!g_tau) return -18;
  if (dU > 0 && !g_U) return -19;
  if (!h->ws || h->ws_bytes < gpp_grad_ws_bytes(N, D, S, dU)) return -1;
  GPP_TRY(gpp_launch_grad_reduce(h->stream, U, N, D, w, sf2, grp, S, kind, d_split, alpha, C, ldc, dU, g_w, g_sf2, g_tau, g_U,
// ... 374 lines not shown
```

gp-plus_amd/csrc/gpp_internal.h:

```cpp
#pragma once
#include <hip/hip_runtime.h>
#include <stdint.h>
#include <stddef.h>
#include <vector>
#include "../../include/gpp.h"

#define GPP_TILE 128
#define GPP_DAG_PLANS 20

struct gpp_handle_s {
  int device;
  hipStream_t stream;
  void* ws;
  size_t ws_bytes;
  hipStream_t panel_stream;
  hipStream_t upd_stream;
  hipStream_t full_stream;
  hipStream_t fill_stream;
  int panel_cus;
  int cu_split;
  hipEvent_t events[16];
  int n_events, ev_next;
  int64_t inv_N;
  int inv_nblocks;
  int64_t inv_o[128], inv_n[128];
  char* panel_flags;
  int panel_next;
  int cap_next;
  hipEvent_t handoff;
  int ncu;
  int coop_panel;
  int panel_fault;
  int panel_timeout_ms;
  struct DagPlan* dag_plans[GPP_DAG_PLANS];
  uint64_t dag_clock;
  struct DagPlan* shard_cur;
  int32_t* shard_info;
  hipEvent_t shard_ready;
  int dag_sched;
  int gemm_tile;
  int split_builds;
  gpp_comm_t comm;
  int comm_rank, comm_nranks;
  void* rccl_comm;
  hipStream_t comm_stream;
  hipEvent_t comm_event;
};
struct GppInvBlocks {
  int64_t N;
  int nblocks;
  decltype(gpp_handle_s::inv_o) o;
  decltype(gpp_handle_s::inv_n) n;
};
inline GppInvBlocks gpp_inv_blocks_save(const gpp_handle_s* h) {
  GppInvBlocks k;
  k.N = h->inv_N;
  k.nblocks = h->inv_nblocks;
  static_assert(sizeof(k.o) == sizeof(h->inv_o) && sizeof(k.n) == sizeof(h->inv_n), "one record");
  for (size_t i = 0; i < sizeof(k.o) / sizeof(k.o[0]); ++i) { k.o[i] = h->inv_o[i]; k.n[i] = h->inv_n[i]; }
  return k;
}
inline void gpp_inv_blocks_restore(gpp_handle_s* h, const GppInvBlocks& k) {
  h->inv_N = k.N;
  h->inv_nblocks = k.nblocks;
  for (size_t i = 0; i < sizeof(k.o) / sizeof(k.o[0]); ++i) { h->inv_o[i] = k.o[i]; h->inv_n[i] = k.n[i]; }
}
extern "C" void gpp_shard_release_comm(gpp_handle_s* h);

struct GppEnv {
  bool coop_panel;
  bool dag_sched;
  bool dag_phased;
  bool shard_list;
  int shard_workers;
  int shard_fill;
  long long shard_timeout_ms;
  int64_t shard_piece_cols;
  bool sharded_force_collectives;
  bool exec_verbose;
  int dag_dump;
  bool dag_check_verbose;
};
const GppEnv& gpp_env();
constexpr int GPP_PANEL_RING = 8;
constexpr int GPP_PANEL_CAP_RING = 16;

#ifdef __HIPCC__
struct GppExpConsts {
  double log2e, ln2_hi, ln2_lo, c[11];
};
__device__ __forceinline__ GppExpConsts gpp_exp_consts() {
  GppExpConsts k = {1.44269504088896338700e+00, 6.93147180369123816490e-01, 1.90821492927058770002e-10,
                    {2.08767569878680989792e-09,
                     2.50521083854417187751e-08,
                     2.75573192239858906526e-07,
                     2.75573192239858906526e-06,
                     2.48015873015873015873e-05,
                     1.98412698412698412698e-04,
                     1.38888888888888888889e-03,
                     8.33333333333333333333e-03,
                     4.16666666666666666667e-02,
                     1.66666666666666666667e-01,
                     0.5}};
  asm volatile("" : "+s"(k.log2e), "+s"(k.ln2_hi), "+s"(k.ln2_lo));
#pragma unroll
  for (int i = 0; i < 10; ++i) asm volatile("" : "+s"(k.c[i]));
  return k;
}
// ... 129 lines not shown
  int workers;
  int fill;
  int fuse;
  int64_t inv_rows;
  int64_t piece_cols;
};
struct DagPlan {
  int64_t N = 0, nb = 0, ld = 0, ldi = 0, ldt = 0, ldk = 0, inv_rows = 0;
  int rank = 0, nranks = 1, workers = 0, fill = 0;
  int c_cph = 0, c_cpt = 0, c_art = 0;
  int piece_tiles = 0, GP = 1;
  std::vector<int> cph_target, cpt_target;
  int flags = 0;
  int B = 0, nt = 0;
  std::vector<int> tb;
  std::vector<GemmArgs> groups;
  std::vector<DagTask> tasks;
  struct Op { int kind, arg, n, lim; };
  std::vector<Op> stream_ops;
  std::vector<int> gate_target;
  std::vector<int> level_first;
  int ncounters = 0;
  int c_pd = 0, c_g1d = 0;
  double sim_ms = 0, sim_busy = 0;
  GemmArgs* d_groups = nullptr;
  GemmArgs* d_groups_abs = nullptr;
  DagTask* d_tasks = nullptr;
  int* d_counters = nullptr;
  unsigned long long* d_trace = nullptr;
  hipEvent_t last_use = nullptr;
  uint64_t stamp = 0;
};
enum { DAG_INV = 1, DAG_SHARD = 4, DAG_BACK = 8 };
DagPlan* gpp_dag_plan(int64_t N, int64_t nb, int64_t ld, int64_t ldi, int64_t ldt, int64_t ldk, int flags, const DagTuning& tune,
                      int rank = 0, int nranks = 1);
DagTuning gpp_dag_default_tuning();
hipError_t gpp_dag_upload(DagPlan* P);
void gpp_dag_free(DagPlan* P);

hipError_t gpp_launch_fill_i32(hipStream_t s, int32_t* p, int n, int32_t value);
size_t gpp_panel_flag_bytes();
int gpp_panel_max_leaves();
hipError_t gpp_launch_panel(hipStream_t s, double* A, int64_t lda, double* Linv, int64_t ldi, int n, int32_t* info, int row_offset,
                            int* flags, int max_wgs, int timeout_ms);
hipError_t gpp_launch_leaf(hipStream_t s, double* A, int64_t lda, double* Linv, int64_t ldi, int n, int32_t* info,
                           int row_offset, int batch = 1, int64_t sA = 0, int64_t sLi = 0);

hipError_t gpp_launch_kernel_build(hipStream_t s, const double* U, int64_t N, int D, const double* w, const double* sf2,
                                   const double* tau, const int32_t* grp, int S, double jitter, int kind, int d_split,
                                   int uplo, double* Ky, int64_t ld, int64_t row0, int64_t nrows, int batch = 1,
                                   int64_t sU = 0, int64_t sK = 0);
hipError_t gpp_launch_cross_kernel(hipStream_t s, const double* Ua, int64_t Ma, const double* Ub, int64_t Nb, int D,
                                   const double* w, const double* sf2, int kind, int d_split, double* Kab, int64_t ld);
hipError_t gpp_launch_post_cov_train(hipStream_t s, const double* Kinv, int64_t ldk, int64_t N, const double* tau, const int32_t* grp,
                                     const double* d, double jitter, double* A, int64_t lda);
hipError_t gpp_launch_sym_rowscale(hipStream_t s, const double* Kinv, int64_t ldk, int64_t N, const double* sv, double* S, int64_t lds);
hipError_t gpp_launch_sym_rowscale_batched(hipStream_t s, const double* Kinv, int64_t ldk, int64_t N, const double* sv, double* S,
                                           int64_t lds, int batch, int64_t sK, int64_t sv_stride, int64_t sS);

int gpp_apply_pieces(int64_t L);
size_t gpp_apply_ws_bytes(int64_t L, int64_t M, int S);
hipError_t gpp_launch_kernel_apply(hipStream_t s, const double* Ua, int64_t M, const double* Ub, int64_t N, int D, const double* w,
                                   const double* sf2, int kind, int d_split, const double* C, int64_t ldc, int S, double beta,
                                   double* Out, int64_t ldo, void* ws, size_t ws_bytes);
hipError_t gpp_launch_rff_apply(hipStream_t s, const double* Ua, int64_t M, int D, const double* Omega, const double* phase, int64_t F,
                                const double* sf2, const double* Theta, int64_t ldt, int S, double beta, double* Out, int64_t ldo,
                                void* ws, size_t ws_bytes);
hipError_t gpp_launch_kernel_apply_grad(hipStream_t s, const double* Ua, int64_t M, const double* Ub, int64_t N, int D, const double* w,
                                        const double* sf2, int kind, int d_split, const double* C, int64_t ldc, int S,
                                        const double* Gbar, int64_t ldg, double beta, double* g_Ua, int64_t ldu, void* ws,
                                        size_t ws_bytes);
hipError_t gpp_launch_rff_apply_grad(hipStream_t s, const double* Ua, int64_t M, int D, const double* Omega, const double* phase,
                                     int64_t F, const double* sf2, const double* Theta, int64_t ldt, int S, const double* Gbar,
                                     int64_t ldg, double beta, double* g_Ua, int64_t ldu, void* ws, size_t ws_bytes);

size_t gpp_append_ws_bytes(int64_t N, int64_t q);

hipError_t gpp_launch_trmv_lower(hipStream_t s, const double* T, int64_t ldt, int64_t N, const double* x, double* y,
                                 int batch = 1, int64_t sT = 0, int64_t sv = 0);
hipError_t gpp_launch_trmv_upper(hipStream_t s, const double* T, int64_t ldt, int64_t N, const double* x, double* y,
                                 int batch = 1, int64_t sT = 0, int64_t sv = 0);
hipError_t gpp_launch_mll_scalars(hipStream_t s, const double* L, int64_t ld, int64_t N, const double* z, double* out3,
                                  int batch = 1, int64_t sL = 0, int64_t sv = 0);
size_t gpp_grad_ws_bytes(int64_t N, int D, int S, int dU);
hipError_t gpp_launch_grad_reduce(hipStream_t s, const double* U, int64_t N, int D, const double* w, const double* sf2,
                                  const int32_t* grp, int S, int kind, int d_split, const double* alpha,
                                  const double* Kinv, int64_t ldk, int dU, double* g_w, double* g_sf2, double* g_tau,
                                  double* g_U, void* ws, size_t ws_bytes, int shard_nb = 0, int shard_rank = 0,
                                  int shard_nranks = 1, int batch = 1, int64_t sU = 0, int64_t sK = 0, int64_t sv = 0,
                                  int shard_cols = 0, const double* beta = nullptr);
hipError_t gpp_launch_loo_scalars(hipStream_t s, const double* Linv, int64_t ldi, int64_t N, const double* alpha, const double* y,
                                  double* d, double* mu, double* s2, double* a, double* sb, double* loo);
hipError_t gpp_launch_loo_scalars_batched(hipStream_t s, const double* Linv, int64_t ldi, int64_t N, const double* alpha,
                                          const double* y, double* d, double* mu, double* s2, double* a, double* sb, double* loo,
                                          int batch, int64_t sLi, int64_t sv);
size_t gpp_lauum_grad_ws_bytes(int64_t N, int D);
hipError_t gpp_launch_grad_finish(hipStream_t s, const double* rec, int64_t nrec, int D, int S, const double* wdiag,
                                  const int32_t* grp, int64_t N, double* g_w, double* g_sf2, double* g_tau);
hipError_t gpp_launch_trmv_lower_cols(hipStream_t s, const double* T, int64_t ldt, int64_t N, const double* x, double* y,
                                      int64_t nb, int rank, int nranks, int trans, void* ws, size_t ws_bytes, int compact = 0);
size_t gpp_trmv_t_ws_bytes(int64_t N);
hipError_t gpp_launch_transpose(hipStream_t s, const double* src, int64_t lds, int64_t rows, int64_t cols, double* dst, int64_t ldd);
size_t gpp_pgrad_ws_bytes(int64_t M, int64_t N, int D, int dA, int dB);
hipError_t gpp_launch_cross_grad(hipStream_t s, const double* Ua, int64_t M, const double* Ub, int64_t N, int D, const double* w,
                                 const double* sf2, int kind, int d_split, const double* gmean, const double* alpha,
                                 const double* gvar, const double* B, int64_t ldb, double* g_Ua, int dA, double* g_Ub, int dB,
                                 double* g_w, double* g_sf2, void* ws, size_t ws_bytes);
hipError_t gpp_launch_predict_reduce(hipStream_t s, const double* Ksn, int64_t lds, const double* V, int64_t ldv,
                                     int64_t M, int64_t N, const double* alpha, const double* kss, double* mean_out,
                                     double* var_out);
```

gp-plus_amd/csrc/gpp_reduce.hip:

```cpp
#include "gpp_internal.h"

#include <algorithm>

typedef double v2d __attribute__((ext_vector_type(2)));

namespace {

__device__ __forceinline__ double wave_sum(double v) {
#pragma unroll
  for (int o = 32; o > 0; o >>= 1) v += __shfl_xor(v, o);
  return v;
}

__global__ __launch_bounds__(256) void gpp_trmv_lower(const double* __restrict__ T, int64_t ldt, int64_t N,
                                                      const double* __restrict__ x, double* __restrict__ y, int64_t sT,
                                                      int64_t sv) {
  const int wave = threadIdx.x >> 6, lane = threadIdx.x & 63;
  const int64_t i = (int64_t)blockIdx.x * 4 + wave;
  if (i >= N) return;
  T += (int64_t)blockIdx.y * sT;
  x += (int64_t)blockIdx.y * sv;
  y += (int64_t)blockIdx.y * sv;
  const double* row = T + i * ldt;
  double acc = 0.0;
  const int64_t len = i + 1;
  const int64_t len2 = len & ~(int64_t)1;
  for (int64_t k = 2 * lane; k < len2; k += 128) {
    const v2d t = *reinterpret_cast<const v2d*>(row + k);
    const v2d xx = *reinterpret_cast<const v2d*>(x + k);
    acc = fma(t.x, xx.x, acc);
    acc = fma(t.y, xx.y, acc);
  }
  if (lane == 0 && (len & 1)) acc = fma(row[len - 1], x[len - 1], acc);
  acc = wave_sum(acc);
  if (lane == 0) y[i] = acc;
}

__global__ __launch_bounds__(256) void gpp_trmv_upper(const double* __restrict__ T, int64_t ldt, int64_t N,
                                                      const double* __restrict__ x, double* __restrict__ y, int64_t sT,
                                                      int64_t sv) {
  const int wave = threadIdx.x >> 6, lane = threadIdx.x & 63;
  const int64_t j = (int64_t)blockIdx.x * 4 + wave;
  if (j >= N) return;
  T += (int64_t)blockIdx.y * sT;
  x += (int64_t)blockIdx.y * sv;
  y += (int64_t)blockIdx.y * sv;
  const double* row = T + j * ldt;
  double acc = 0.0;
  int64_t k0 = j;
  if (k0 & 1) {
    if (lane == 0) acc = fma(row[k0], x[k0], acc);
    ++k0;
  }
  const int64_t nvec = (N - k0) >> 1;
  for (int64_t v = lane; v < nvec; v += 64) {
    const v2d t = *reinterpret_cast<const v2d*>(row + k0 + 2 * v);
    const v2d xx = *reinterpret_cast<const v2d*>(x + k0 + 2 * v);
    acc = fma(t.x, xx.x, acc);
    acc = fma(t.y, xx.y, acc);
  }
  if (lane == 0 && ((N - k0) & 1)) acc = fma(row[N - 1], x[N - 1], acc);
  acc = wave_sum(acc);
  if (lane == 0) y[j] = acc;
}

__global__ __launch_bounds__(256) void gpp_trmv_lower_cols(const double* __restrict__ T, int64_t ldt, int64_t N,
                                                           const double* __restrict__ x, double* __restrict__ y, int64_t nb,
                                                           int rank, int nranks, int compact) {
  const int wave = threadIdx.x >> 6, lane = threadIdx.x & 63;
  const int64_t i = (int64_t)blockIdx.x * 4 + wave;
  if (i >= N) return;
  const double* row = T + i * ldt;
  double acc = 0.0;
  int64_t q = 0;
  for (int64_t c0 = (int64_t)rank * nb; c0 <= i; c0 += (int64_t)nranks * nb, ++q) {
    const int64_t c1 = (c0 + nb < i + 1) ? c0 + nb : i + 1;
    const int64_t len = c1 - c0, len2 = len & ~(int64_t)1;
    const double* seg = row + (compact ? q * nb : c0);
    for (int64_t k = 2 * lane; k < len2; k += 128) {
      const v2d t = *reinterpret_cast<const v2d*>(seg + k);
      const v2d xx = *reinterpret_cast<const v2d*>(x + c0 + k);
      acc = fma(t.x, xx.x, acc);
      acc = fma(t.y, xx.y, acc);
    }
    if (lane == 0 && (len & 1)) acc = fma(seg[len - 1], x[c1 - 1], acc);
  }
  acc = wave_sum(acc);
  if (lane == 0) y[i] = acc;
}

constexpr int TRT_CHUNKS = 16;
__global__ __launch_bounds__(256) void gpp_trmv_lower_t_cols(const double* __restrict__ T, int64_t ldt, int64_t N,
                                                             const double* __restrict__ x, double* __restrict__ part, int64_t nb,
                                                             int rank, int nranks, int64_t chunk, int compact) {
  __shared__ double red[4][64];
  const int wave = threadIdx.x >> 6, lane = threadIdx.x & 63;
  const int64_t k0 = (int64_t)blockIdx.x * 64, k = k0 + lane;
  const bool owned = (int)((k0 / nb) % nranks) == rank;
  double acc = 0.0;
  const int64_t r0 = (int64_t)blockIdx.y * chunk, r1 = (r0 + chunk < N) ? r0 + chunk : N;
  if (owned && k < N && r1 > k0) {
    int64_t i = (r0 > k0 ? r0 : k0) + wave;
    const double* p = T + (compact ? ((k0 / nb) / nranks) * nb + (k0 % nb) + lane : k);
    for (; i + 28 < r1; i += 32) {
      double t[8], xv[8];
#pragma unroll
      for (int u = 0; u < 8; ++u) {
        t[u] = p[(i + 4 * u) * ldt];
        xv[u] = x[i + 4 * u];
      }
#pragma unroll
      for (int u = 0; u < 8; ++u) acc = (i + 4 * u >= k) ? fma(t[u], xv[u], acc) : acc;
    }
    for (; i < r1; i += 4)
      if (i >= k) acc = fma(p[i * ldt], x[i], acc);
  }
  red[wave][lane] = acc;
  __syncthreads();
  if (wave == 0 && k < N) part[(int64_t)blockIdx.y * N + k] = (red[0][lane] + red[1][lane]) + (red[2][lane] + red[3][lane]);
}
__global__ __launch_bounds__(256) void gpp_trmv_lower_t_finish(const double* __restrict__ part, int64_t N, int chunks,
                                                               double* __restrict__ y) {
  const int64_t k = (int64_t)blockIdx.x * 256 + threadIdx.x;
  if (k >= N) return;
  double s = 0.0;
  for (int r = 0; r < chunks; ++r) s += part[(int64_t)r * N + k];
  y[k] = s;
}

__global__ __launch_bounds__(1024) void gpp_mll_scalars(const double* __restrict__ L, int64_t ld, int64_t N,
                                                        const double* __restrict__ z, double* __restrict__ out3, int64_t sL,
                                                        int64_t sv) {
  __shared__ double sq[16], sl[16];
  L += (int64_t)blockIdx.x * sL;
  z += (int64_t)blockIdx.x * sv;
  out3 += 3 * (int64_t)blockIdx.x;
  double q = 0.0, l = 0.0;
  for (int64_t i = threadIdx.x; i < N; i += 1024) {
    const double zi = z[i];
    q = fma(zi, zi, q);
    l += log(L[i * ld + i]);
  }
  q = wave_sum(q);
  l = wave_sum(l);
  const int wave = threadIdx.x >> 6, lane = threadIdx.x & 63;
  if (lane == 0) {
    sq[wave] = q;
    sl[wave] = l;
  }
  __syncthreads();
  if (threadIdx.x == 0) {
    double qq = 0.0, ll = 0.0;
    for (int w = 0; w < 16; ++w) {
      qq += sq[w];
      ll += sl[w];
    }
    ll *= 2.0;
    out3[0] = qq;
    out3[1] = ll;
    out3[2] = -0.5 * (qq + ll + (double)N * 1.8378770664093454835606594728112);
  }
}

__global__ __launch_bounds__(256) void gpp_loo_rows(const double* __restrict__ Linv, int64_t ldi, int64_t N,
                                                    const double* __restrict__ alpha, const double* __restrict__ y,
                                                    double* __restrict__ d, double* __restrict__ mu, double* __restrict__ s2,
                                                    double* __restrict__ a, double* __restrict__ sb, int64_t sLi, int64_t sv) {
  const int wave = threadIdx.x >> 6, lane = threadIdx.x & 63;
  const int64_t i = (int64_t)blockIdx.x * 4 + wave;
  if (i >= N) return;
  const int64_t vo = (int64_t)blockIdx.y * sv;
  const double* row = Linv + (int64_t)blockIdx.y * sLi + i * ldi;
  double acc = 0.0;
  int64_t k0 = i;
  if (k0 & 1) {
    if (lane == 0) acc = row[k0] * row[k0];
    ++k0;
  }
  const int64_t nvec = (N - k0) >> 1;
#pragma unroll 4
  for (int64_t v = lane; v < nvec; v += 64) {
    const v2d t = *reinterpret_cast<const v2d*>(row + k0 + 2 * v);
    acc = fma(t.x, t.x, acc);
    acc = fma(t.y, t.y, acc);
  }
  if (lane == 0 && ((N - k0) & 1)) acc = fma(row[N - 1], row[N - 1], acc);
  acc = wave_sum(acc);
  if (lane == 0) {
    const int64_t o = vo + i;
    const double di = acc, al = alpha[o], inv = 1.0 / di;
    d[o] = di;
    if (mu) mu[o] = y[o] - al * inv;
    if (s2) s2[o] = inv;
    if (a) a[o] = -al * inv;
    if (sb) sb[o] = sqrt(0.5 * inv + 0.5 * (al * inv) * (al * inv));
  }
}

__global__ __launch_bounds__(1024) void gpp_loo_value(const double* __restrict__ d, const double* __restrict__ alpha, int64_t N,
                                                      double* __restrict__ out, int64_t sv) {
  __shared__ double sp[16];
  d += (int64_t)blockIdx.x * sv;
  alpha += (int64_t)blockIdx.x * sv;
  out += blockIdx.x;
  double s = 0.0;
  for (int64_t i = threadIdx.x; i < N; i += 1024) {
    const double di = d[i], al = alpha[i];
    s += 0.5 * log(di) - 0.5 * al * al / di;
  }
  s = wave_sum(s);
  const int wave = threadIdx.x >> 6, lane = threadIdx.x & 63;
  if (lane == 0) sp[wave] = s;
  __syncthreads();
  if (threadIdx.x == 0) {
    double t = 0.0;
    for (int w = 0; w < 16; ++w) t += sp[w];
    out[0] = t - 0.5 * (double)N * 1.8378770664093454835606594728112;
  }
}

constexpr int GT = 64;
constexpr int GD_MAX = 64;
constexpr int GS_MAX = 64;
constexpr int G_WGS = 2048;

__device__ __forceinline__ void tile_from_index(int64_t t, int64_t& ti, int64_t& tj) {
  int64_t r = (int64_t)((sqrt(8.0 * (double)t + 1.0) - 1.0) * 0.5);
  while ((r + 1) * (r + 2) / 2 <= t) ++r;
  while (r * (r + 1) / 2 > t) --r;
  ti = r;
  tj = t - r * (r + 1) / 2;
}

template <int DT, bool MAT, bool HASU, bool LOO = false>
__global__ __launch_bounds__(256) void gpp_grad_tiles(const double* __restrict__ U, int64_t N, int D,
                                                      const double* __restrict__ w, const double* __restrict__ sf2p,
                                                      int kind, int d_split, const double* __restrict__ alpha, const double* __restrict__ Kinv,
                                                      int64_t ldk, int dU, int64_t ntiles, int shard_nb, int shard_rank,
                                                      int shard_nranks, int shard_cols, int64_t sU, int64_t sK, int64_t sv, int64_t ws_stride,
                                                      double* __restrict__ rec ,
                                                      double* __restrict__ wdiag ,
                                                      double* __restrict__ gUpart ,
                                                      const double* __restrict__ beta ) {
  {
// ... 451 lines not shown
          gBpart[((int64_t)t * N + j0 + tid) * dB + d] =
              2.0 * wd * ((colred[tid] + colred[GT + tid]) + (colred[2 * GT + tid] + colred[3 * GT + tid]));
        __syncthreads();
      }
    }
  }
  __syncthreads();
  for (int e = tid; e < dA * GT; e += 256) {
    const int d = e / GT, r = e - d * GT;
    if (i0 + r < M) gApart[((int64_t)c * M + i0 + r) * dA + d] = accA[e];
  }
  const int nrec = D + 1;
  const int64_t wg = t * CN + c;
  for (int q = 0; q < nrec; ++q) {
    double v = my_sf2;
    if (q < D) v = (lane == 0) ? wacc[wave * DT + q] : 0.0;
    __syncthreads();
    red[tid] = v;
    __syncthreads();
    for (int o = 128; o > 0; o >>= 1) {
      if (tid < o) red[tid] += red[tid + o];
      __syncthreads();
    }
    if (tid == 0) rec[wg * nrec + q] = red[0];
  }
}

__global__ __launch_bounds__(256) void gpp_pgrad_finish(const double* __restrict__ rec, int nwg, int D, double* __restrict__ g_w,
                                                        double* __restrict__ g_sf2) {
  __shared__ double red[256];
  const int q = blockIdx.x, nrec = D + 1, tid = threadIdx.x;
  double v = 0.0;
  for (int b = tid; b < nwg; b += 256) v += rec[(int64_t)b * nrec + q];
  red[tid] = v;
  __syncthreads();
  for (int o = 128; o > 0; o >>= 1) {
    if (tid < o) red[tid] += red[tid + o];
    __syncthreads();
  }
  if (tid == 0) {
    if (q < D && g_w) g_w[q] = red[0];
    else if (q == D && g_sf2) g_sf2[0] = red[0];
  }
}

__global__ __launch_bounds__(256) void gpp_predict_rows(const double* __restrict__ Ksn, int64_t lds, const double* __restrict__ V,
                                                        int64_t ldv, int64_t M, int64_t N, const double* __restrict__ alpha,
                                                        const double* __restrict__ kss, double* __restrict__ mean_out,
                                                        double* __restrict__ var_out) {
  const int wave = threadIdx.x >> 6, lane = threadIdx.x & 63;
  const int64_t a = (int64_t)blockIdx.x * 4 + wave;
  if (a >= M) return;
  double m = 0.0, q = 0.0;
  const double* kr = Ksn + a * lds;
  for (int64_t j = lane; j < N; j += 64) m = fma(kr[j], alpha[j], m);
  if (V) {
    const double* vr = V + a * ldv;
    for (int64_t j = lane; j < N; j += 64) q = fma(vr[j], vr[j], q);
  }
  m = wave_sum(m);
  q = wave_sum(q);
  if (lane == 0) {
    mean_out[a] = m;
    if (V && var_out) var_out[a] = kss[a] - q;
  }
}

}

hipError_t gpp_launch_trmv_lower(hipStream_t s, const double* T, int64_t ldt, int64_t N, const double* x, double* y,
                                 int batch, int64_t sT, int64_t sv) {
  if (N <= 0 || batch <= 0) return hipSuccess;
  hipLaunchKernelGGL(gpp_trmv_lower, dim3((unsigned)((N + 3) / 4), (unsigned)batch), dim3(256), 0, s, T, ldt, N, x, y, sT, sv);
  return hipGetLastError();
}

hipError_t gpp_launch_trmv_upper(hipStream_t s, const double* T, int64_t ldt, int64_t N, const double* x, double* y,
                                 int batch, int64_t sT, int64_t sv) {
  if (N <= 0 || batch <= 0) return hipSuccess;
  hipLaunchKernelGGL(gpp_trmv_upper, dim3((unsigned)((N + 3) / 4), (unsigned)batch), dim3(256), 0, s, T, ldt, N, x, y, sT, sv);
  return hipGetLastError();
}

size_t gpp_trmv_t_ws_bytes(int64_t N) { return (size_t)TRT_CHUNKS * (size_t)N * sizeof(double); }

hipError_t gpp_launch_trmv_lower_cols(hipStream_t s, const double* T, int64_t ldt, int64_t N, const double* x, double* y,
                                      int64_t nb, int rank, int nranks, int trans, void* ws, size_t ws_bytes, int compact) {
  if (N <= 0) return hipSuccess;
  if (nb < 64 || nb % 64 != 0 || nranks < 1 || rank < 0 || rank >= nranks) return hipErrorInvalidValue;
  if (trans) {
    if (!ws || ws_bytes < gpp_trmv_t_ws_bytes(N)) return hipErrorInvalidValue;
    const int64_t chunk = (((N + TRT_CHUNKS - 1) / TRT_CHUNKS) + 31) / 32 * 32;
    double* part = reinterpret_cast<double*>(ws);
    hipLaunchKernelGGL(gpp_trmv_lower_t_cols, dim3((unsigned)((N + 63) / 64), TRT_CHUNKS), dim3(256), 0, s, T, ldt, N, x, part, nb,
                       rank, nranks, chunk, compact);
    hipLaunchKernelGGL(gpp_trmv_lower_t_finish, dim3((unsigned)((N + 255) / 256)), dim3(256), 0, s, part, N, TRT_CHUNKS, y);
  } else
    hipLaunchKernelGGL(gpp_trmv_lower_cols, dim3((unsigned)((N + 3) / 4)), dim3(256), 0, s, T, ldt, N, x, y, nb, rank, nranks, compact);
  return hipGetLastError();
}

hipError_t gpp_launch_mll_scalars(hipStream_t s, const double* L, int64_t ld, int64_t N, const double* z, double* out3,
                                  int batch, int64_t sL, int64_t sv) {
  if (batch <= 0) return hipSuccess;
  hipLaunchKernelGGL(gpp_mll_scalars, dim3((unsigned)batch), dim3(1024), 0, s, L, ld, N, z, out3, sL, sv);
  return hipGetLastError();
}

hipError_t gpp_launch_loo_scalars_batched(hipStream_t s, const double* Linv, int64_t ldi, int64_t N, const double* alpha,
                                          const double* y, double* d, double* mu, double* s2, double* a, double* sb, double* loo,
                                          int batch, int64_t sLi, int64_t sv) {
  if (batch <= 0) return hipSuccess;
  if (batch > 65535) return hipErrorInvalidValue;
  if (N > 0)
    hipLaunchKernelGGL(gpp_loo_rows, dim3((unsigned)((N + 3) / 4), (unsigned)batch), dim3(256), 0, s, Linv, ldi, N, alpha, y, d, mu,
                       s2, a, sb, sLi, sv);
  if (loo) hipLaunchKernelGGL(gpp_loo_value, dim3((unsigned)batch), dim3(1024), 0, s, d, alpha, N, loo, sv);
  return hipGetLastError();
}

hipError_t gpp_launch_loo_scalars(hipStream_t s, const double* Linv, int64_t ldi, int64_t N, const double* alpha, const double* y,
                                  double* d, double* mu, double* s2, double* a, double* sb, double* loo) {
  return gpp_launch_loo_scalars_batched(s, Linv, ldi, N, alpha, y, d, mu, s2, a, sb, loo, 1, 0, 0);
}

size_t gpp_grad_ws_bytes(int64_t N, int D, int S, int dU) {
  (void)S;
  const int64_t T = (N + GT - 1) / GT;
  return (size_t)G_WGS * (D + 1) * sizeof(double) + (size_t)N * sizeof(double) +
         (size_t)T * N * (dU > 0 ? dU : 0) * sizeof(double) + 256;
}

hipError_t gpp_launch_grad_reduce(hipStream_t s, const double* U, int64_t N, int D, const double* w, const double* sf2,
                                  const int32_t* grp, int S, int kind, int d_split, const double* alpha,
                                  const double* Kinv, int64_t ldk, int dU, double* g_w, double* g_sf2, double* g_tau,
                                  double* g_U, void* ws, size_t ws_bytes, int shard_nb, int shard_rank, int shard_nranks,
                                  int batch, int64_t sU, int64_t sK, int64_t sv, int shard_cols, const double* beta) {
  if (kind < 0 || kind > 2) return hipErrorInvalidValue;
  if (batch < 1 || batch > 65535) return hipErrorInvalidValue;
  if (shard_nranks > 1 && (shard_nb < GT || shard_nb % GT != 0 || shard_rank < 0 || shard_rank >= shard_nranks))
    return hipErrorInvalidValue;
  if (D > GD_MAX || D < 1 || S > GS_MAX || S < 1 || dU > D || dU < 0) return hipErrorInvalidValue;
  if (ws_bytes < (size_t)batch * gpp_grad_ws_bytes(N, D, S, dU)) return hipErrorInvalidValue;
  const int64_t ws_stride = (int64_t)(gpp_grad_ws_bytes(N, D, S, dU) / sizeof(double));
  const int T = (int)((N + GT - 1) / GT);
  const int64_t ntiles = (int64_t)T * (T + 1) / 2;
  const int nwg = (int)(ntiles < G_WGS ? ntiles : G_WGS);
  double* rec = reinterpret_cast<double*>(ws);
  double* wdiag = rec + (size_t)G_WGS * (D + 1);
  double* gUpart = wdiag + N;
  if (shard_nranks > 1) {
    hipError_t e = hipMemsetAsync(ws, 0, (size_t)batch * ws_stride * sizeof(double), s);
    if (e != hipSuccess) return e;
  }
  auto launch = [&](auto kern) {
    hipLaunchKernelGGL(kern, dim3(nwg, batch), dim3(256), 0, s, U, N, D, w, sf2, kind, d_split, alpha, Kinv, ldk, dU, ntiles,
                       shard_nb, shard_rank, shard_nranks, shard_cols, sU, sK, sv, ws_stride, rec, wdiag, gUpart, beta);
  };
  const bool mat = kind != 0, hasu = dU > 0, loo = beta != nullptr;
#define GPP_GT2(DT, LOO)                                                                                             \
  (mat ? (hasu ? launch(gpp_grad_tiles<DT, true, true, LOO>) : launch(gpp_grad_tiles<DT, true, false, LOO>))         \
       : (hasu ? launch(gpp_grad_tiles<DT, false, true, LOO>) : launch(gpp_grad_tiles<DT, false, false, LOO>)))
#define GPP_GT(DT) (loo ? GPP_GT2(DT, true) : GPP_GT2(DT, false))
  if (D <= 8) GPP_GT(8);
  else if (D <= 16) GPP_GT(16);
  else if (D <= 32) GPP_GT(32);
// ... 105 lines not shown
```

gp-plus_amd/linalg.py:

```python
from __future__ import annotations

import math
import threading
from contextlib import contextmanager, nullcontext
from dataclasses import dataclass
from typing import Dict, Optional, Tuple

import torch

from .backend import (KIND_MATERN32, KIND_RBF, UPLO_FULL, UPLO_UPPER, GppContext, get_context, row_stride, rows_buffer,
                      square_buffer)
from .psd_safe import inputs_nan_probe, psd_safe
from . import settings

__all__ = ["KernelSpec", "exact_mll", "ExactMLLFunction", "exact_loo", "ExactLOOFunction", "loo_moments", "exact_cv", "ExactCVFunction",
           "cv_moments", "EvalWorkspace", "dense_kernel", "cross_kernel",
           "FactorCache", "factorize", "append_to_cache", "GradientFactorCache", "append_gradients_to_cache",
           "predict_from_gradient_cache", "dense_log_prob", "predict_mean", "predict_var", "predictive_cov_upper",
           "train_post_cov_upper", "mvn_root", "mvn_draw"]


@dataclass
class KernelSpec:
    w: torch.Tensor
# ... 88 lines not shown


def _factor(ctx: GppContext, ws: EvalWorkspace, U, w, sf2, tau, grp, kind, d_split, after=None) -> float:
    if torch.cuda.is_current_stream_capturing():
        if ws.N >= LOOKAHEAD_MIN_N:
            raise RuntimeError("graph capture of the evaluation is limited to the single-stream factorisation (N < 3840)")
        ctx.kernel_build(U, w, sf2, tau, grp, ws.A, jitter=0.0, kind=kind, d_split=d_split, uplo=UPLO_UPPER)
        ctx.potrf(ws.A, ws.Li, ws.info, ws.Ki)
        if after is not None:
            after()
        return 0.0

    def attempt(jit):
        if ws.N >= LOOKAHEAD_MIN_N:
            torch.cuda.current_stream(ctx.index).synchronize()
        with _stage("kernel_build"):
            pass
        with _stage("potrf"):
            ctx.build_potrf(U, w, sf2, tau, grp, ws.A, ws.Li, ws.info, ws.Ki, jitter=jit, kind=kind, d_split=d_split)
        ws.info_host.copy_(ws.info, non_blocking=True)
        ws.info_event.record(torch.cuda.current_stream(ctx.index))
        if after is not None:
            after()
        ws.info_event.synchronize()
        return int(ws.info_host[0])

    return psd_safe(ctx, attempt, inputs_nan_probe(U, w, sf2, tau))


def _operands(U, w, sf2, tau, grp):
    dev = U.device
    Ud, wd, sd, td = _as_f64(U.detach(), dev), _as_f64(w.detach(), dev), _as_f64(sf2.detach().reshape(1), dev), \
        _as_f64(tau.detach().reshape(-1), dev)
    if grp is not None and grp.dtype != torch.int32:
        grp = grp.to(torch.int32)
    return Ud, wd, sd, td, grp


def _eval_operands(ctx, U, w, sf2, tau, mean, y, grp, dU):
    Ud, wd, sd, td, grp = _operands(U, w, sf2, tau, grp)
    need = ctx.needs_input_grad
    ctx.in_dtypes = (U.dtype, w.dtype, sf2.dtype, tau.dtype, mean.dtype, y.dtype)
    ctx.shapes = (sf2.shape, tau.shape)
    return Ud, wd, sd, td, grp, td.numel(), any(need[:6]), need[0] and dU > 0


def _eval_backward(ctx, grad_out, g_w, g_s, g_t, g_Ud, g_mean):
    need = ctx.needs_input_grad
    go = grad_out.to(torch.float64)
    g_U = None
    if need[0]:
        g_U = torch.zeros(g_mean.shape[0], g_w.shape[0], dtype=torch.float64, device=g_mean.device)
        if g_Ud is not None:
            g_U[:, :g_Ud.shape[1]] = g_Ud
    dt = ctx.in_dtypes
    sf2_shape, tau_shape = ctx.shapes
    return (None if g_U is None else (go * g_U).to(dt[0]),
            (go * g_w).to(dt[1]) if need[1] else None,
            (go * g_s).reshape(sf2_shape).to(dt[2]) if need[2] else None,
            (go * g_t).reshape(tau_shape).to(dt[3]) if need[3] else None,
            (go * g_mean).to(dt[4]) if need[4] else None,
            (-go * g_mean).to(dt[5]) if need[5] else None)


def _exact_forward(fn, ctx, U, w, sf2, tau, mean, y, grp, kind, d_split, dU, slot):
    gctx = get_context(U.device)
    with torch.cuda.device(U.device):
        if not fn.capturable and torch.cuda.is_current_stream_capturing():
            raise NotImplementedError(f"{getattr(fn, 'what', 'the leave-one-out objective')} is not available inside a graph capture")
        dev = U.device
        N, D = U.shape
        Ud, wd, sd, td, grp, S, need_grad, need_U = _eval_operands(ctx, U, w, sf2, tau, mean, y, grp, dU)
        ws = get_workspace(gctx, N, slot)
        ws.epoch += 1
        torch.sub(_as_f64(y.detach(), dev), _as_f64(mean.detach(), dev), out=ws.r)
        g_w = g_s = g_t = g_Ud = None
        if need_grad:
            g_w = torch.empty(D, dtype=torch.float64, device=dev)
            g_s = torch.empty(1, dtype=torch.float64, device=dev)
            g_t = torch.empty(S, dtype=torch.float64, device=dev)
            g_Ud = torch.empty(N, dU, dtype=torch.float64, device=dev) if need_U else None
        ops, grads = (Ud, wd, sd, grp, S), (dU if need_U else 0, g_w, g_s, g_t, g_Ud)

        def rest():
            with _stage("trtri"):
                gctx.trtri(ws.A, ws.Li, ws.Ki)
            with _stage("mll_reduce"):
                gctx.mll_reduce(ws.A, ws.Li, ws.r, ws.z, ws.out3)
            if need_grad or fn.value_needs_alpha:
                with _stage("alpha"):
                    gctx.alpha(ws.Li, ws.z, ws.alpha)
            fn.tail(gctx, ws, need_grad, ops, grads, kind, d_split)

        _factor(gctx, ws, Ud, wd, sd, td, grp, kind, d_split, after=rest)
        value, g_mean = fn.result(ws, need_grad)
        ctx.saved = (g_w, g_s, g_t, g_Ud, g_mean)
        return value


class ExactMLLFunction(torch.autograd.Function):

    capturable, value_needs_alpha = True, False

    @staticmethod
    def forward(ctx, U, w, sf2, tau, mean, y, grp, kind, d_split, dU, slot):
        return _exact_forward(ExactMLLFunction, ctx, U, w, sf2, tau, mean, y, grp, kind, d_split, dU, slot)

    @staticmethod
    def tail(gctx, ws, need_grad, ops, grads, kind, d_split):
        if not need_grad:
            return
        fused = False
        with _stage("lauum"):
            if ws.N > FUSED_GRAD_MIN_N:
                fused = gctx.lauum_grad(ws.Li, *ops, ws.alpha, *grads[:4], kind=kind)
            if not fused:
                gctx.lauum(ws.Li, ws.Ki)
        with _stage("grad_reduce"):
            if not fused:
                gctx.grad_reduce(*ops, ws.alpha, ws.Ki, *grads, kind=kind, d_split=d_split)

    @staticmethod
    def result(ws, need_grad):
        return ws.out3[2].clone(), (ws.alpha.clone() if need_grad else None)

    @staticmethod
    def backward(ctx, grad_out):
        return _eval_backward(ctx, grad_out, *ctx.saved) + (None,) * 5


def exact_mll(U: torch.Tensor, spec: KernelSpec, tau: torch.Tensor, mean: torch.Tensor, y: torch.Tensor,
              grp: Optional[torch.Tensor] = None, n_grad_dims: Optional[int] = None, slot: Optional[int] = None) -> torch.Tensor:
    if slot is None:
        slot = current_slot()
    if n_grad_dims is None:
        n_grad_dims = U.shape[1] if U.requires_grad else 0
    shard = settings.sharded_evaluation.value()
    if shard is not None:
        from .sharded import sharded_mll
        return sharded_mll(U, spec.w, spec.sf2, tau, mean, y, grp, spec.kind, spec.d_split, int(n_grad_dims),
                           group=shard.get("group"), nb=int(shard.get("nb", 1024)))
    return ExactMLLFunction.apply(U, spec.w, spec.sf2, tau, mean, y, grp, spec.kind, spec.d_split, int(n_grad_dims), slot)


class ExactLOOFunction(torch.autograd.Function):

    capturable, value_needs_alpha = False, True

    @staticmethod
    def forward(ctx, U, w, sf2, tau, mean, y, grp, kind, d_split, dU, slot):
        return _exact_forward(ExactLOOFunction, ctx, U, w, sf2, tau, mean, y, grp, kind, d_split, dU, slot)

    @staticmethod
    def tail(gctx, ws, need_grad, ops, grads, kind, d_split):
        N, lv = ws.N, ws.loo_vectors()
        with _stage("loo_scalars"):
            gctx.loo_scalars(ws.Li, ws.alpha, None, lv.d, a=lv.a, sqrtb=lv.sb, loo=lv.val)
        if not need_grad:
            return
        with _stage("loo_beta"):
            gctx.mll_reduce(ws.A, ws.Li, lv.a, lv.z, lv.out3)
            gctx.alpha(ws.Li, lv.z, lv.beta)
        with _stage("lauum"):
            gctx.lauum(ws.Li, ws.Ki)
        with _stage("sym_rowscale"):
            gctx.sym_rowscale(ws.Ki, lv.sb, ws.A)
        with _stage("loo_gemm"):
            gctx.gemm(1, 0, N, N, N, 1.0, ws.A, ws.A, 0.0, ws.Li, c_tri=1)
        with _stage("loo_grad_reduce"):
            gctx.loo_grad_reduce(*ops, ws.alpha, lv.beta, ws.Li, *grads, kind=kind, d_split=d_split)

    @staticmethod
    def result(ws, need_grad):
        lv = ws.loo_vectors()
        return lv.val[0].clone(), (lv.beta.neg() if need_grad else None)

    @staticmethod
    def backward(ctx, grad_out):
        return _eval_backward(ctx, grad_out, *ctx.saved) + (None,) * 5


def exact_loo(U: torch.Tensor, spec: KernelSpec, tau: torch.Tensor, mean: torch.Tensor, y: torch.Tensor,
              grp: Optional[torch.Tensor] = None, n_grad_dims: Optional[int] = None, slot: Optional[int] = None) -> torch.Tensor:
    if slot is None:
        slot = current_slot()
    if n_grad_dims is None:
        n_grad_dims = U.shape[1] if U.requires_grad else 0
    if settings.sharded_evaluation.value() is not None:
        raise NotImplementedError("the leave-one-out objective is not available under settings.sharded_evaluation")
    return ExactLOOFunction.apply(U, spec.w, spec.sf2, tau, mean, y, grp, spec.kind, spec.d_split, int(n_grad_dims), slot)


class _CVEvaluation:

    capturable, value_needs_alpha, what = False, True, "the cross-validation objective"

    def __init__(self, folds):
        self.folds, self.terms, self.infos = folds, None, None

    def tail(self, gctx, ws, need_grad, ops, grads, kind, d_split):
        from .cv import fold_gradient_factors, fold_solves
        N, lv = ws.N, ws.loo_vectors()
        with _stage("cv_folds"):
            a, _, self.terms, self.infos, kept = fold_solves(gctx, ws.Li, ws.alpha, self.folds, keep_factors=need_grad)
        if not need_grad:
            return
        lv.a.copy_(a)
        with _stage("cv_beta"):
            gctx.mll_reduce(ws.A, ws.Li, lv.a, lv.z, lv.out3)
            gctx.alpha(ws.Li, lv.z, lv.beta)
        with _stage("lauum"):
            gctx.lauum(ws.Li, ws.Ki)
        with _stage("sym_rowscale"):
            gctx.sym_rowscale(ws.Ki, torch.ones(N, dtype=torch.float64, device=ws.A.device), ws.A)
        with _stage("cv_rows"):
            for b, Li_b, z, na, out3 in kept:
                G = fold_gradient_factors(b, Li_b, z, na, out3)
                gctx.cv_rows(G, b.idx, b.off, ws.A, ws.Li[b.base:b.base + b.rows])
                del G
        del kept
        with _stage("cv_gemm"):
            gctx.gemm(1, 0, N, N, N, 1.0, ws.Li, ws.Li, 0.0, ws.A, c_tri=1)
        with _stage("loo_grad_reduce"):
            gctx.loo_grad_reduce(*ops, ws.alpha, lv.beta, ws.A, *grads, kind=kind, d_split=d_split)

    def result(self, ws, need_grad):
        from .cv import check_infos
        check_infos(self.infos, self.folds)
        value = self.terms.sum() - 0.5 * ws.N * math.log(2.0 * math.pi)
        return value, (ws.loo_vectors().beta.neg() if need_grad else None)


class ExactCVFunction(torch.autograd.Function):

    @staticmethod
    def forward(ctx, U, w, sf2, tau, mean, y, grp, kind, d_split, dU, slot, folds):
        return _exact_forward(_CVEvaluation(folds), ctx, U, w, sf2, tau, mean, y, grp, kind, d_split, dU, slot)

    @staticmethod
    def backward(ctx, grad_out):
        return _eval_backward(ctx, grad_out, *ctx.saved) + (None,) * 6


def exact_cv(U: torch.Tensor, spec: KernelSpec, tau: torch.Tensor, mean: torch.Tensor, y: torch.Tensor, folds,
             grp: Optional[torch.Tensor] = None, n_grad_dims: Optional[int] = None, slot: Optional[int] = None) -> torch.Tensor:
    from .cv import FoldIndex
    folds = FoldIndex.make(folds, U.shape[0])
    if slot is None:
        slot = current_slot()
    if n_grad_dims is None:
        n_grad_dims = U.shape[1] if U.requires_grad else 0
    if settings.sharded_evaluation.value() is not None:
        raise NotImplementedError("the cross-validation objective is not available under settings.sharded_evaluation")
    return ExactCVFunction.apply(U, spec.w, spec.sf2, tau, mean, y, grp, spec.kind, spec.d_split, int(n_grad_dims), slot, folds)


@torch.no_grad()
def dense_kernel(U: torch.Tensor, spec: KernelSpec, tau: Optional[torch.Tensor] = None,
                 grp: Optional[torch.Tensor] = None, jitter: float = 0.0) -> torch.Tensor:
    dev = U.device
    gctx = get_context(dev)
    N = U.shape[0]
    out = square_buffer(N, dev)
    gctx.kernel_build(_as_f64(U, dev), _as_f64(spec.w, dev), _as_f64(spec.sf2.reshape(1), dev),
                      None if tau is None else _as_f64(tau.reshape(-1), dev),
                      None if grp is None else grp.to(torch.int32), out, jitter=jitter, kind=spec.kind,
                      d_split=spec.d_split, uplo=UPLO_FULL)
    return out


@torch.no_grad()
def cross_kernel(Ua: torch.Tensor, Ub: torch.Tensor, spec: KernelSpec) -> torch.Tensor:
    dev = Ua.device
    gctx = get_context(dev)
    M, N = Ua.shape[0], Ub.shape[0]
    out = rows_buffer(M, N, dev)
    gctx.cross_kernel(_as_f64(Ua, dev), _as_f64(Ub, dev), _as_f64(spec.w, dev), _as_f64(spec.sf2.reshape(1), dev), out,
                      kind=spec.kind, d_split=spec.d_split)
# ... 786 lines not shown
```

include/gpp.h:

```cpp
#ifndef GPP_H
#define GPP_H

#include <stddef.h>
#include <stdint.h>

#ifdef __cplusplus
extern "C" {
#endif

typedef struct gpp_handle_s* gpp_handle_t;

#define GPP_KIND_RBF      0
#define GPP_KIND_MATERN32 1
#define GPP_KIND_MATERN52 2

#define GPP_UPLO_FULL  0
#define GPP_UPLO_LOWER 1
#define GPP_UPLO_UPPER 2

#define GPP_OP_MLL_EVAL 0
#define GPP_OP_PREDICT  1
#define GPP_OP_PREDICT_GRAD 2
#define GPP_OP_APPLY 3
#define GPP_OP_APPLY_GRAD 4
#define GPP_OP_APPEND 5
#define GPP_OP_POST_CROSS 6
#define GPP_OP_POST_CROSS_MIN 7
#define GPP_OP_POINT_GRAM 8

const char* gpp_version(void);

int gpp_create(gpp_handle_t* out, int device);
int gpp_destroy(gpp_handle_t h);
int gpp_set_stream(gpp_handle_t h, void* stream);
int gpp_internal_stream(gpp_handle_t h, int which, void** out);
#define GPP_OPT_COOP_PANEL 1
#define GPP_OPT_PANEL_FAULT 2
#define GPP_OPT_PANEL_TIMEOUT_MS 3
#define GPP_OPT_EXEC_SCHED 4
#define GPP_OPT_DAG_SCHED 5
#define GPP_OPT_GEMM_TILE 6
#define GPP_INFO_PANEL_TIMEOUT (1 << 30)
#define GPP_INFO_EXEC_TIMEOUT ((1 << 30) | (1 << 29))
int gpp_set_option(gpp_handle_t h, int option, int value);
size_t gpp_workspace_bytes(gpp_handle_t h, int op, int64_t N, int64_t M, int D, int S);
int gpp_set_workspace(gpp_handle_t h, void* ws, size_t bytes);

int gpp_kernel_build(gpp_handle_t h, const double* U, int64_t N, int D, const double* w, const double* sf2,
                     const double* tau, const int32_t* grp, int S, double jitter, int kind, int d_split,
                     int uplo, double* Ky, int64_t ld, int64_t row0, int64_t nrows);

int gpp_cross_kernel(gpp_handle_t h, const double* Ua, int64_t Ma, const double* Ub, int64_t Nb, int D,
                     const double* w, const double* sf2, int kind, int d_split, double* Kab, int64_t ld);

int gpp_kernel_apply(gpp_handle_t h, const double* Ua, int64_t M, const double* Ub, int64_t N, int D, const double* w,
                     const double* sf2, int kind, int d_split, const double* C, int64_t ldc, int S, double beta, double* Out,
                     int64_t ldo);
int gpp_rff_apply(gpp_handle_t h, const double* Ua, int64_t M, int D, const double* Omega, const double* phase, int64_t F,
                  const double* sf2, const double* Theta, int64_t ldt, int S, double beta, double* Out, int64_t ldo);

int gpp_kernel_apply_grad(gpp_handle_t h, const double* Ua, int64_t M, const double* Ub, int64_t N, int D, const double* w,
                          const double* sf2, int kind, int d_split, const double* C, int64_t ldc, int S, const double* Gbar,
                          int64_t ldg, double beta, double* g_Ua, int64_t ldu);
int gpp_rff_apply_grad(gpp_handle_t h, const double* Ua, int64_t M, int D, const double* Omega, const double* phase, int64_t F,
                       const double* sf2, const double* Theta, int64_t ldt, int S, const double* Gbar, int64_t ldg, double beta,
                       double* g_Ua, int64_t ldu);

int gpp_potrf(gpp_handle_t h, double* A, int64_t N, int64_t ld, double* Linv, int64_t ldi, int32_t* info_dev);
int gpp_potrf_ws(gpp_handle_t h, double* A, int64_t N, int64_t ld, double* Linv, int64_t ldi, double* T, int64_t ldt,
                 int32_t* info_dev);

int gpp_build_potrf_ws(gpp_handle_t h, const double* U, int64_t N, int D, const double* w, const double* sf2, const double* tau,
                       const int32_t* grp, int S, double jitter, int kind, int d_split, double* A, int64_t ld, double* Linv,
                       int64_t ldi, double* T, int64_t ldt, int32_t* info_dev);

int gpp_trtri(gpp_handle_t h, const double* U, int64_t N, int64_t ld, double* Linv, int64_t ldi, double* T, int64_t ldt);

int gpp_lauum(gpp_handle_t h, const double* Linv, int64_t N, int64_t ldi, double* Kinv, int64_t ldk);

#define GPP_NOT_SUPPORTED 2001
#define GPP_NO_WORKSPACE 2002
int gpp_lauum_grad(gpp_handle_t h, const double* Linv, int64_t N, int64_t ldi, const double* U, int D, const double* w,
                   const double* sf2, const int32_t* grp, int S, int kind, int dU, const double* alpha, double* g_w,
                   double* g_sf2, double* g_tau);

int gpp_post_cov_train(gpp_handle_t h, const double* Kinv, int64_t N, int64_t ldk, const double* tau, const int32_t* grp, int S,
                       const double* d, double jitter, double* A, int64_t lda);

int gpp_syrk_rows(gpp_handle_t h, const double* Urow, int64_t ldu, double* C, int64_t ldc, int64_t Nt, int64_t K, int64_t nb,
                  int64_t first_block, int rank, int nranks);

int gpp_gemm_lower_cols(gpp_handle_t h, const double* A, int64_t lda, const double* B, int64_t ldb, double* C, int64_t ldc,
                        int64_t M, int64_t K, double alpha, double beta, int64_t nb, int64_t first_block, int rank, int nranks,
                        int64_t row0, int64_t row1, int compact);

int gpp_shard_list_begin(gpp_handle_t h, int64_t N, int64_t nb, int rank, int nranks, double* A, int64_t ld, double* Kc, double* Lc,
                         int64_t ldc, double* D, double* W0, double* W1, double* W2, int64_t ldw, int32_t* info, int workers,
                         int* used);
int64_t gpp_shard_piece_cols(void);
int gpp_shard_list_gate(gpp_handle_t h, void* stream, int tail, int k);
int gpp_shard_list_signal(gpp_handle_t h, void* stream, int tail, int k);
int gpp_shard_list_end(gpp_handle_t h);

int gpp_shard_back_list(gpp_handle_t h, int64_t N, int64_t nb, int rank, int nranks, const double* A, int64_t ld, double* Kc, double* Lc,
                        int64_t ldc, const double* D, int32_t* info, int workers, int* used);

enum { GPP_COMM_SUM_F64 = 0, GPP_COMM_MAX_I32 = 1 };
#define GPP_SHARD_UNSUPPORTED 2000
typedef struct gpp_comm {
  void* user;
  int (*bcast)(void* user, void* dev_buf, size_t bytes, int root, void* stream);
  int (*allreduce)(void* user, void* dev_buf, size_t count, int kind, void* stream);
} gpp_comm_t;
typedef struct gpp_shard_buffers {
  double* A; int64_t ld;
  double* Kc; double* Lc; int64_t ldc;
  double* D;
  double* W0; double* W1; double* W2; int64_t ldw;
  double* msg;
  double* z; double* alpha; double* r;
  double* flat;
  double* out3; int32_t* info;
} gpp_shard_buffers_t;
int gpp_set_comm(gpp_handle_t h, const gpp_comm_t* comm, int rank, int nranks);
int gpp_comm_unique_id(void* out128);
int gpp_comm_init_rccl(gpp_handle_t h, const void* unique_id128, int rank, int nranks);
size_t gpp_shard_buffer_doubles(int64_t N, int64_t nb, int rank, int nranks, int which);
int gpp_shard_eval(gpp_handle_t h, int64_t N, int64_t nb, const double* U, int D, const double* w, const double* sf2, const double* tau,
                   const int32_t* grp, int S, int kind, int d_split, double jitter, int dU, int need_grad, const gpp_shard_buffers_t* b,
                   int32_t* info_host);

typedef struct gpp_push* gpp_push_t;
#define GPP_PUSH_HANDLE_BYTES 128
int gpp_push_create(int device, int rank, int nranks, int64_t slot_bytes, gpp_push_t* out, void* handle_out);
int gpp_push_connect(gpp_push_t p, const void* handles );
int gpp_push_send(gpp_push_t p, void* after_stream, int64_t seq, int32_t* status, int code, int nparts, const void* const* src,
                  const int64_t* spitch, const int64_t* offset, const int64_t* dpitch, const int64_t* width, const int64_t* height);
int gpp_push_recv(gpp_push_t p, void* stream, int64_t seq, int32_t* status, int code, int nparts, void* const* dst, const int64_t* dpitch,
                  const int64_t* offset, const int64_t* spitch, const int64_t* width, const int64_t* height);
int gpp_push_ack(gpp_push_t p, void* stream, int64_t seq);
int gpp_push_info(gpp_push_t p, int64_t* slot_bytes, int* flag_kind );
int gpp_push_destroy(gpp_push_t p, int stage);

int gpp_trmv_lower_cols(gpp_handle_t h, const double* T, int64_t ldt, int64_t N, const double* x, double* y, int64_t nb, int rank,
                        int nranks, int trans, int compact);

int gpp_mll_scalars(gpp_handle_t h, const double* U, int64_t ld, int64_t N, const double* z, double* out3);

int gpp_lauum_rows(gpp_handle_t h, const double* Linv, int64_t N, int64_t ldi, double* Kinv, int64_t ldk, int rank, int nranks);

int gpp_lauum_rows_range(gpp_handle_t h, const double* Linv, int64_t N, int64_t ldi, double* Kinv, int64_t ldk, int rank,
                         int nranks, int64_t row0, int64_t row1);

int gpp_transpose(gpp_handle_t h, const double* src, int64_t lds, int64_t rows, int64_t cols, double* dst, int64_t ldd);

int gpp_mll_reduce(gpp_handle_t h, const double* U, int64_t ld, const double* Linv, int64_t ldi, int64_t N,
                   const double* r, double* z, double* out3);

int gpp_alpha(gpp_handle_t h, const double* Linv, int64_t ldi, int64_t N, const double* z, double* alpha);

int gpp_grad_reduce(gpp_handle_t h, const double* U, int64_t N, int D, const double* w, const double* sf2,
                    const int32_t* grp, int S, int kind, int d_split, const double* alpha, const double* Kinv,
                    int64_t ldk, int dU, double* g_w, double* g_sf2, double* g_tau, double* g_U);

int gpp_loo_scalars(gpp_handle_t h, const double* Linv, int64_t ldi, int64_t N, const double* alpha, const double* y, double* d,
                    double* mu, double* s2, double* a, double* sqrtb, double* loo);

int gpp_sym_rowscale(gpp_handle_t h, const double* Kinv, int64_t N, int64_t ldk, const double* s, double* S, int64_t lds);

int gpp_loo_grad_reduce(gpp_handle_t h, const double* U, int64_t N, int D, const double* w, const double* sf2,
                        const int32_t* grp, int S, int kind, int d_split, const double* alpha, const double* beta,
                        const double* C, int64_t ldc, int dU, double* g_w, double* g_sf2, double* g_tau, double* g_U);

int gpp_grad_reduce_rows(gpp_handle_t h, const double* U, int64_t N, int D, const double* w, const double* sf2,
                         const int32_t* grp, int S, int kind, int d_split, const double* alpha, const double* Kinv,
                         int64_t ldk, int dU, int64_t nb, int rank, int nranks, double* g_w, double* g_sf2, double* g_tau,
                         double* g_U);

int gpp_grad_reduce_cols(gpp_handle_t h, const double* U, int64_t N, int D, const double* w, const double* sf2,
                         const int32_t* grp, int S, int kind, int d_split, const double* alpha, const double* Kinv,
                         int64_t ldk, int dU, int64_t nb, int rank, int nranks, double* g_w, double* g_sf2, double* g_tau,
                         double* g_U, int compact);

int gpp_predict(gpp_handle_t h, const double* Linv, int64_t ldi, int64_t N, const double* alpha, const double* Ksn,
                int64_t lds, int64_t M, const double* kss, double* V, int64_t ldv, double* mean_out, double* var_out);

int gpp_predict_tn(gpp_handle_t h, const double* Linv, int64_t ldi, int64_t N, const double* z, const double* Kns, int64_t ldk,
                   int64_t M, const double* kss, double* V, int64_t ldv, double* mean_out, double* var_out);

int gpp_cross_grad(gpp_handle_t h, const double* Ua, int64_t M, const double* Ub, int64_t N, int D, const double* w,
                   const double* sf2, int kind, int d_split, const double* gmean, const double* alpha, const double* gvar,
                   const double* B, int64_t ldb, double* g_Ua, int dA, double* g_Ub, int dB, double* g_w, double* g_sf2);

int gpp_gemm(gpp_handle_t h, int transA, int transB, int64_t M, int64_t N, int64_t K, double alpha, const double* A,
             int64_t lda, const double* B, int64_t ldb, double beta, double* C, int64_t ldc, int a_mask, int b_mask,
             int klo_mode, int khi_mode, int c_tri);

int gpp_gemm_batched(gpp_handle_t h, int transA, int transB, int64_t M, int64_t N, int64_t K, double alpha, const double* A,
                     int64_t lda, int64_t sA, const double* B, int64_t ldb, int64_t sB, double beta, double* C, int64_t ldc,
                     int64_t sC, int batch, int a_mask, int b_mask, int klo_mode, int khi_mode, int c_tri);

int gpp_kernel_build_batched(gpp_handle_t h, const double* U, int64_t sU, int64_t N, int D, const double* w, const double* sf2,
                             const double* tau, const int32_t* grp, int S, double jitter, int kind, int d_split, int uplo,
                             double* Ky, int64_t ld, int64_t sK, int batch);
int gpp_potrf_batched(gpp_handle_t h, double* A, int64_t N, int64_t ld, int64_t sA, double* Linv, int64_t ldi, int64_t sLi,
                      int32_t* info_dev, int batch);
int gpp_trtri_batched(gpp_handle_t h, const double* U, int64_t N, int64_t ld, int64_t sA, double* Linv, int64_t ldi,
                      int64_t sLi, double* T, int64_t ldt, int64_t sT, int batch);
int gpp_lauum_batched(gpp_handle_t h, const double* Linv, int64_t N, int64_t ldi, int64_t sLi, double* Kinv, int64_t ldk,
                      int64_t sK, int batch);
int gpp_mll_reduce_batched(gpp_handle_t h, const double* U, int64_t ld, int64_t sA, const double* Linv, int64_t ldi,
                           int64_t sLi, int64_t N, const double* r, double* z, int64_t sv, double* out3, int batch);
int gpp_alpha_batched(gpp_handle_t h, const double* Linv, int64_t ldi, int64_t sLi, int64_t N, const double* z, double* alpha,
                      int64_t sv, int batch);
int gpp_grad_reduce_batched(gpp_handle_t h, const double* U, int64_t sU, int64_t N, int D, const double* w, const double* sf2,
                            const int32_t* grp, int S, int kind, int d_split, const double* alpha, int64_t sv,
                            const double* Kinv, int64_t ldk, int64_t sK, int dU, double* g_w, double* g_sf2, double* g_tau,
                            double* g_U, int batch);

int gpp_loo_scalars_batched(gpp_handle_t h, const double* Linv, int64_t ldi, int64_t sLi, int64_t N, const double* alpha,
                            const double* y, double* d, double* mu, double* s2, double* a, double* sqrtb, int64_t sv, double* loo,
                            int batch);
int gpp_sym_rowscale_batched(gpp_handle_t h, const double* Kinv, int64_t N, int64_t ldk, int64_t sK, const double* s, int64_t sv,
                             double* S, int64_t lds, int64_t sS, int batch);
int gpp_loo_grad_reduce_batched(gpp_handle_t h, const double* U, int64_t sU, int64_t N, int D, const double* w, const double* sf2,
                                const int32_t* grp, int S, int kind, int d_split, const double* alpha, const double* beta,
                                int64_t sv, const double* C, int64_t ldc, int64_t sC, int dU, double* g_w, double* g_sf2,
                                double* g_tau, double* g_U, int batch);

int gpp_cv_blocks(gpp_handle_t h, const double* Linv, int64_t ldi, int64_t N, const int32_t* idx, const int32_t* off, int nfolds,
                  int mp, double* B, int64_t ldb, int64_t sB);
int gpp_cv_rows(gpp_handle_t h, const double* G, int64_t ldg, int64_t sG, const int32_t* idx, const int32_t* off, int nfolds,
                const double* Psq, int64_t ldp, int64_t N, double* S, int64_t lds);

int gpp_chol_append(gpp_handle_t h, double* A, int64_t ld, double* Linv, int64_t ldi, int64_t N, int64_t q, const double* k,
                    int64_t ldk, const double* C, int64_t ldc, const double* rq, double* z, double* alpha, int32_t* info_dev);

int gpp_post_cross_sq(gpp_handle_t h, const double* Uc, int64_t Mc, const double* Ur, int64_t Mr, int D, const double* w,
                      const double* sf2, int kind, int d_split, const double* Vc, int64_t ldc, const double* Vr, int64_t ldr,
                      int64_t K, int vt, const double* omega, double* out);

// ... 18 lines not shown
```

Baseline: 7.712 evals/s.

## Skip mirror writes in trtri and fuse mll reduce with alpha solve

Adds a lower-only trtri variant that omits the mirrored upper-triangle stores of the final recursion levels, recording them so a later call can fill them in by transpose if needed. Adds a fused kernel that computes z = Linv r row-wise and accumulates the transposed product alpha = Linv^T z from the same row tiles into per-chunk partial buffers, with a finish kernel that sums partials and computes the MLL scalars. The exact MLL path now uses both, which removes the separate alpha pass over Linv and some mirror write traffic. The cost is extra workspace for the triangular partial buffers, and any later consumer that reads the upper mirror must depend on complete_mirror being called.

```diff
diff --git a/gp-plus_amd/_lib.py b/gp-plus_amd/_lib.py
--- a/gp-plus_amd/_lib.py
+++ b/gp-plus_amd/_lib.py
@@ -38,6 +38,8 @@
     "gpp_build_potrf_ws": (c_int, [c_void_p, c_void_p, c_int64, c_int, c_void_p, c_void_p, c_void_p, c_void_p, c_int, c_double, c_int,
                                    c_int, c_void_p, c_int64, c_void_p, c_int64, c_void_p, c_int64, c_void_p]),
     "gpp_trtri": (c_int, [c_void_p, c_void_p, c_int64, c_int64, c_void_p, c_int64, c_void_p, c_int64]),
+    "gpp_trtri_lower": (c_int, [c_void_p, c_void_p, c_int64, c_int64, c_void_p, c_int64, c_void_p, c_int64]),
+    "gpp_trtri_complete_mirror": (c_int, [c_void_p, c_void_p, c_int64, c_int64]),
     "gpp_lauum": (c_int, [c_void_p, c_void_p, c_int64, c_int64, c_void_p, c_int64]),
     "gpp_lauum_grad": (c_int, [c_void_p, c_void_p, c_int64, c_int64, c_void_p, c_int, c_void_p, c_void_p, c_void_p, c_int, c_int, c_int,
                                c_void_p, c_void_p, c_void_p, c_void_p]),
@@ -79,6 +81,7 @@
     "gpp_transpose": (c_int, [c_void_p, c_void_p, c_int64, c_int64, c_int64, c_void_p, c_int64]),
     "gpp_mll_reduce": (c_int, [c_void_p, c_void_p, c_int64, c_void_p, c_int64, c_int64, c_void_p, c_void_p, c_void_p]),
     "gpp_alpha": (c_int, [c_void_p, c_void_p, c_int64, c_int64, c_void_p, c_void_p]),
+    "gpp_mll_reduce_alpha": (c_int, [c_void_p, c_void_p, c_int64, c_void_p, c_int64, c_int64, c_void_p, c_void_p, c_void_p, c_void_p]),
     "gpp_grad_reduce": (c_int, [c_void_p, c_void_p, c_int64, c_int, c_void_p, c_void_p, c_void_p, c_int, c_int, c_int,
                                 c_void_p, c_void_p, c_int64, c_int, c_void_p, c_void_p, c_void_p, c_void_p]),
     "gpp_loo_scalars": (c_int, [c_void_p, c_void_p, c_int64, c_int64, c_void_p, c_void_p, c_void_p, c_void_p, c_void_p, c_void_p, c_void_p,
diff --git a/gp-plus_amd/backend.py b/gp-plus_amd/backend.py
--- a/gp-plus_amd/backend.py
+++ b/gp-plus_amd/backend.py
@@ -314,6 +314,17 @@
               "gpp_trtri")
 
     @_on_own_device
+    def trtri_lower(self, U, Linv, T):
+        self._stream()
+        check(self.lib.gpp_trtri_lower(self.h, U.data_ptr(), U.shape[0], _ld(U), Linv.data_ptr(), _ld(Linv), T.data_ptr(), _ld(T)),
+              "gpp_trtri_lower")
+
+    @_on_own_device
+    def complete_mirror(self, Linv):
+        self._stream()
+        check(self.lib.gpp_trtri_complete_mirror(self.h, Linv.data_ptr(), Linv.shape[0], _ld(Linv)), "gpp_trtri_complete_mirror")
+
+    @_on_own_device
     def lauum(self, Linv, Kinv):
         self._stream()
         check(self.lib.gpp_lauum(self.h, Linv.data_ptr(), Linv.shape[0], _ld(Linv), Kinv.data_ptr(), _ld(Kinv)), "gpp_lauum")
@@ -455,6 +466,15 @@
         self._stream()
         check(self.lib.gpp_mll_reduce(self.h, L.data_ptr(), _ld(L), Linv.data_ptr(), _ld(Linv), L.shape[0], r.data_ptr(),
                                       z.data_ptr(), out3.data_ptr()), "gpp_mll_reduce")
+
+    @_on_own_device
+    def mll_reduce_alpha(self, L, Linv, r, z, out3, alpha):
+        for t, n in ((r, "r"), (z, "z"), (out3, "out3"), (alpha, "alpha")):
+            _need(t, torch.float64, n)
+        self.ensure_workspace(OP_MLL_EVAL, L.shape[0], 0, 1, 1)
+        self._stream()
+        check(self.lib.gpp_mll_reduce_alpha(self.h, L.data_ptr(), _ld(L), Linv.data_ptr(), _ld(Linv), L.shape[0], r.data_ptr(),
+                                            z.data_ptr(), out3.data_ptr(), alpha.data_ptr()), "gpp_mll_reduce_alpha")
 
     @_on_own_device
     def alpha(self, Linv, z, alpha):
diff --git a/gp-plus_amd/csrc/gpp_api.hip b/gp-plus_amd/csrc/gpp_api.hip
--- a/gp-plus_amd/csrc/gpp_api.hip
+++ b/gp-plus_amd/csrc/gpp_api.hip
@@ -173,13 +173,17 @@
   return launch_panel_at(h, b, o, n, max_wgs);
 }
 
-template <typename Skip>
+struct MirrorAll {
+  bool operator()(int64_t, int64_t) const { return true; }
+  void omitted(int64_t, int64_t, int64_t) const {}
+};
+template <typename Skip, typename Need = MirrorAll>
 hipError_t trtri_level(hipStream_t st, const double* U, int64_t ld, double* Linv, int64_t ldi, double* T, int64_t ldt,
                        int64_t base, int64_t n, int64_t s, Skip skip, int mbatch = 1, int64_t msU = 0, int64_t msLi = 0,
-                       int64_t msT = 0, int g1_tile = 0, hipEvent_t before_g2 = nullptr) {
+                       int64_t msT = 0, int g1_tile = 0, hipEvent_t before_g2 = nullptr, Need need = Need()) {
   const int64_t npairs_full = n / (2 * s);
   const int64_t rem = n - npairs_full * 2 * s;
-  auto launch = [&](int64_t o, int64_t m2, int batch) -> hipError_t {
+  auto launch = [&](int64_t o, int64_t m2, int batch, bool mirror) -> hipError_t {
     const int64_t pstride_U = 2 * s * (ld + 1), pstride_I = 2 * s * (ldi + 1), pstride_T = 2 * s * (ldt + 1);
     GemmArgs g1 = mk(U + o * ld + (o + s), ld, Linv + o * ldi + o, ldi, T + (o + s) * ldt + o, ldt, m2, s, s, 1.0, 0.0);
     g1.b_mask = 2; g1.klo_mode = 2; g1.col_major = 1;
@@ -196,7 +200,8 @@
                      m2, -1.0, 0.0);
     g2.a_mask = 1; g2.khi_mode = 1; g2.row_reverse = 1;
     g2.sA = pstride_I; g2.sB = pstride_T; g2.sC = pstride_I;
-    g2.C2 = Linv + o * ldi + (o + s); g2.ldc2 = ldi; g2.sC2 = pstride_I;
+    g2.C2 = mirror ? Linv + o * ldi + (o + s) : nullptr; g2.ldc2 = ldi; g2.sC2 = pstride_I;
+    if (!mirror) need.omitted(o, s, m2);
     g2.batch2 = mbatch; g2.zA = msLi; g2.zB = msT; g2.zC = msLi; g2.zC2 = msLi;
     g2.batch_fast = 1;
     return gpp_launch_gemm(st, 2, g2, batch);
@@ -204,14 +209,15 @@
   int64_t p = 0;
   while (p < npairs_full) {
     if (skip(base + 2 * s * p)) { ++p; continue; }
-    int64_t q = p;
-    while (q < npairs_full && !skip(base + 2 * s * q)) ++q;
-    hipError_t e = launch(base + 2 * s * p, s, (int)(q - p));
+    const bool mirror = need(base + 2 * s * p, s);
+    int64_t q = p + 1;
+    while (mirror && q < npairs_full && !skip(base + 2 * s * q) && need(base + 2 * s * q, s)) ++q;
+    hipError_t e = launch(base + 2 * s * p, s, (int)(q - p), mirror);
     if (e != hipSuccess) return e;
     p = q;
   }
   if (rem > s && !skip(base + npairs_full * 2 * s)) {
-    hipError_t e = launch(base + npairs_full * 2 * s, rem - s, 1);
+    hipError_t e = launch(base + npairs_full * 2 * s, rem - s, 1, need(base + npairs_full * 2 * s, s));
     if (e != hipSuccess) return e;
   }
   return hipSuccess;
@@ -734,6 +740,9 @@
   h->ev_next = 0;
   h->inv_N = 0;
   h->inv_nblocks = 0;
+  h->mir_Li = nullptr;
+  h->mir_N = h->mir_ldi = 0;
+  h->mir_n = 0;
   h->panel_flags = nullptr;
   h->panel_next = 0;
   h->coop_panel = gpp_env().coop_panel ? 1 : 0;
@@ -1029,7 +1038,7 @@
 size_t gpp_workspace_bytes(gpp_handle_t h, int op, int64_t N, int64_t M, int D, int S) {
   (void)h;
   if (op == GPP_OP_MLL_EVAL) {
-    return std::max({gpp_grad_ws_bytes(N, D, S, D), gpp_trmv_t_ws_bytes(N), gpp_lauum_grad_ws_bytes(N, D)}) + 256;
+    return std::max({gpp_grad_ws_bytes(N, D, S, D), gpp_trmv_t_ws_bytes(N), gpp_lauum_grad_ws_bytes(N, D), gpp_mll_alpha_ws_bytes(N)}) + 256;
   }
   if (op == GPP_OP_PREDICT) return 256;
   if (op == GPP_OP_PREDICT_GRAD) return gpp_pgrad_ws_bytes(M, N, D, D, S) + 256;
@@ -1265,7 +1274,27 @@
   return r == -9 ? -7 : r;
 }
 
-int gpp_trtri(gpp_handle_t h, const double* U, int64_t N, int64_t ld, double* Linv, int64_t ldi, double* T, int64_t ldt) {
+extern "C++" {
+struct MirrorNeeded {
+  gpp_handle_s* h;
+  int64_t N;
+  bool operator()(int64_t b, int64_t s) const {
+    if (h->mir_n >= GPP_MIR_MAX) return true;
+    for (int64_t s2 = 2 * s; s2 < N; s2 *= 2)
+      if (b % (2 * s2) >= s2) return true;
+    return false;
+  }
+  void omitted(int64_t b, int64_t s, int64_t m2) const {
+    h->mir_b[h->mir_n] = b;
+    h->mir_s[h->mir_n] = s;
+    h->mir_m[h->mir_n] = m2;
+    ++h->mir_n;
+  }
+};
+
+template <typename Need>
+static int trtri_impl(gpp_handle_t h, const double* U, int64_t N, int64_t ld, double* Linv, int64_t ldi, double* T, int64_t ldt,
+                      Need need) {
   if (!h) return -1;
   if (N < 0) return -3;
   if (int r = check_mat(U, ld, N, 2)) return r;
@@ -1281,9 +1310,39 @@
         if (b >= h->inv_o[i] && h->inv_o[i] + h->inv_n[i] == N && b + s < N) return true;
       return false;
     };
-    GPP_TRY(trtri_level(h->stream, U, ld, Linv, ldi, T, ldt, 0, N, s, skip));
+    GPP_TRY(trtri_level(h->stream, U, ld, Linv, ldi, T, ldt, 0, N, s, skip, 1, 0, 0, 0, 0, nullptr, need));
   }
   h->inv_N = 0;
+  return 0;
+}
+}
+
+int gpp_trtri(gpp_handle_t h, const double* U, int64_t N, int64_t ld, double* Linv, int64_t ldi, double* T, int64_t ldt) {
+  const int r = trtri_impl(h, U, N, ld, Linv, ldi, T, ldt, MirrorAll{});
+  if (r == 0 && h->mir_Li == Linv) h->mir_n = 0;
+  return r;
+}
+
+int gpp_trtri_lower(gpp_handle_t h, const double* U, int64_t N, int64_t ld, double* Linv, int64_t ldi, double* T, int64_t ldt) {
+  if (!h) return -1;
+  h->mir_Li = Linv;
+  h->mir_N = N;
+  h->mir_ldi = ldi;
+  h->mir_n = 0;
+  return trtri_impl(h, U, N, ld, Linv, ldi, T, ldt, MirrorNeeded{h, N});
+}
+
+int gpp_trtri_complete_mirror(gpp_handle_t h, double* Linv, int64_t N, int64_t ldi) {
+  if (!h) return -1;
+  if (h->mir_n == 0) return 0;
+  if (Linv != h->mir_Li) return -2;
+  if (N != h->mir_N) return -3;
+  if (ldi != h->mir_ldi) return -4;
+  for (int i = 0; i < h->mir_n; ++i) {
+    const int64_t b = h->mir_b[i], s = h->mir_s[i], m = h->mir_m[i];
+    GPP_TRY(gpp_launch_transpose(h->stream, Linv + (b + s) * ldi + b, ldi, m, s, Linv + b * ldi + (b + s), ldi));
+  }
+  h->mir_n = 0;
   return 0;
 }
 
@@ -1465,6 +1524,21 @@
   if (!out3) return -9;
   GPP_TRY(gpp_launch_trmv_lower(h->stream, Linv, ldi, N, r, z));
   GPP_TRY(gpp_launch_mll_scalars(h->stream, U, ld, N, z, out3));
+  return 0;
+}
+
+int gpp_mll_reduce_alpha(gpp_handle_t h, const double* U, int64_t ld, const double* Linv, int64_t ldi, int64_t N, const double* r,
+                         double* z, double* out3, double* alpha) {
+  if (!h) return -1;
+  if (N < 0) return -6;
+  if (int q = check_mat(U, ld, N, 2)) return q;
+  if (int q = check_mat(Linv, ldi, N, 4)) return q;
+  if (!r || !aligned16(r)) return -7;
+  if (!z) return -8;
+  if (!out3) return -9;
+  if (!alpha) return -10;
+  if (N > 0 && (!h->ws || h->ws_bytes < gpp_mll_alpha_ws_bytes(N))) return GPP_NO_WORKSPACE;
+  GPP_TRY(gpp_launch_mll_reduce_alpha(h->stream, U, ld, Linv, ldi, N, r, z, out3, alpha, h->ws, h->ws_bytes));
   return 0;
 }
 
diff --git a/gp-plus_amd/csrc/gpp_internal.h b/gp-plus_amd/csrc/gpp_internal.h
--- a/gp-plus_amd/csrc/gpp_internal.h
+++ b/gp-plus_amd/csrc/gpp_internal.h
@@ -8,6 +8,7 @@
 #define GPP_TILE 128
 #define GPP_DAG_PLANS 20
 
+constexpr int GPP_MIR_MAX = 64;
 struct gpp_handle_s {
   int device;
   hipStream_t stream;
@@ -24,6 +25,10 @@
   int64_t inv_N;
   int inv_nblocks;
   int64_t inv_o[128], inv_n[128];
+  const double* mir_Li;
+  int64_t mir_N, mir_ldi;
+  int mir_n;
+  int64_t mir_b[GPP_MIR_MAX], mir_s[GPP_MIR_MAX], mir_m[GPP_MIR_MAX];
   char* panel_flags;
   int panel_next;
   int cap_next;
@@ -319,6 +324,9 @@
                                  int batch = 1, int64_t sT = 0, int64_t sv = 0);
 hipError_t gpp_launch_mll_scalars(hipStream_t s, const double* L, int64_t ld, int64_t N, const double* z, double* out3,
                                   int batch = 1, int64_t sL = 0, int64_t sv = 0);
+hipError_t gpp_launch_mll_reduce_alpha(hipStream_t s, const double* L, int64_t ld, const double* T, int64_t ldt, int64_t N,
+                                       const double* r, double* z, double* out3, double* alpha, void* ws, size_t ws_bytes);
+size_t gpp_mll_alpha_ws_bytes(int64_t N);
 size_t gpp_grad_ws_bytes(int64_t N, int D, int S, int dU);
 hipError_t gpp_launch_grad_reduce(hipStream_t s, const double* U, int64_t N, int D, const double* w, const double* sf2,
                                   const int32_t* grp, int S, int kind, int d_split, const double* alpha,
diff --git a/gp-plus_amd/csrc/gpp_reduce.hip b/gp-plus_amd/csrc/gpp_reduce.hip
--- a/gp-plus_amd/csrc/gpp_reduce.hip
+++ b/gp-plus_amd/csrc/gpp_reduce.hip
@@ -10,6 +10,20 @@
 #pragma unroll
   for (int o = 32; o > 0; o >>= 1) v += __shfl_xor(v, o);
   return v;
+}
+
+__device__ __forceinline__ double trmv_row_dot(const double* __restrict__ row, const double* __restrict__ x, int64_t len, int lane) {
+  double acc = 0.0;
+  const int64_t len2 = len & ~(int64_t)1;
+#pragma unroll 4
+  for (int64_t k = 2 * lane; k < len2; k += 128) {
+    const v2d t = *reinterpret_cast<const v2d*>(row + k);
+    const v2d xx = *reinterpret_cast<const v2d*>(x + k);
+    acc = fma(t.x, xx.x, acc);
+    acc = fma(t.y, xx.y, acc);
+  }
+  if (lane == 0 && (len & 1)) acc = fma(row[len - 1], x[len - 1], acc);
+  return wave_sum(acc);
 }
 
 __global__ __launch_bounds__(256) void gpp_trmv_lower(const double* __restrict__ T, int64_t ldt, int64_t N,
@@ -128,13 +142,8 @@
   y[k] = s;
 }
 
-__global__ __launch_bounds__(1024) void gpp_mll_scalars(const double* __restrict__ L, int64_t ld, int64_t N,
-                                                        const double* __restrict__ z, double* __restrict__ out3, int64_t sL,
-                                                        int64_t sv) {
-  __shared__ double sq[16], sl[16];
-  L += (int64_t)blockIdx.x * sL;
-  z += (int64_t)blockIdx.x * sv;
-  out3 += 3 * (int64_t)blockIdx.x;
+__device__ __forceinline__ void mll_scalars_block(const double* __restrict__ L, int64_t ld, int64_t N, const double* __restrict__ z,
+                                                  double* __restrict__ out3, double* sq , double* sl ) {
   double q = 0.0, l = 0.0;
   for (int64_t i = threadIdx.x; i < N; i += 1024) {
     const double zi = z[i];
@@ -160,6 +169,79 @@
     out3[1] = ll;
     out3[2] = -0.5 * (qq + ll + (double)N * 1.8378770664093454835606594728112);
   }
+}
+__global__ __launch_bounds__(1024) void gpp_mll_scalars(const double* __restrict__ L, int64_t ld, int64_t N,
+                                                        const double* __restrict__ z, double* __restrict__ out3, int64_t sL,
+                                                        int64_t sv) {
+  __shared__ double sq[16], sl[16];
+  mll_scalars_block(L + (int64_t)blockIdx.x * sL, ld, N, z + (int64_t)blockIdx.x * sv, out3 + 3 * (int64_t)blockIdx.x, sq, sl);
+}
+
+constexpr int MA_ROWS = 32;
+__host__ __device__ inline int64_t ma_slot(int64_t c) { return 16 * c * (c + 1); }
+
+__global__ __launch_bounds__(1024) __attribute__((amdgpu_waves_per_eu(8, 8))) void gpp_mll_alpha_rows(const double* __restrict__ T, int64_t ldt, int64_t N,
+                                                           const double* __restrict__ r, double* __restrict__ z,
+                                                           double* __restrict__ part, int64_t C) {
+  __shared__ double zs[MA_ROWS];
+  const int wave = threadIdx.x >> 6, lane = threadIdx.x & 63;
+  for (int half = 0; half < 2; ++half) {
+    const int64_t c = half == 0 ? C - 1 - (int64_t)blockIdx.x : (int64_t)blockIdx.x;
+    if (half == 1 && c >= C - 1 - (int64_t)blockIdx.x) break;
+    const int64_t i0 = c * MA_ROWS, i1 = (i0 + MA_ROWS < N) ? i0 + MA_ROWS : N;
+    for (int q = wave; q < MA_ROWS; q += 16) {
+      const int64_t i = i0 + q;
+      double v = 0.0;
+      if (i < i1) v = trmv_row_dot(T + i * ldt, r, i + 1, lane);
+      if (lane == 0) {
+        zs[q] = v;
+        if (i < i1) z[i] = v;
+      }
+    }
+    __syncthreads();
+    const int nr = (int)(i1 - i0);
+    double* slot = part + ma_slot(c);
+    for (int64_t k = 2 * (int64_t)threadIdx.x; k < i1; k += 2048) {
+      const double* p = T + i0 * ldt + k;
+      double a0 = 0.0, a1 = 0.0;
+      if (k + 1 <= i0) {
+#pragma unroll 8
+        for (int q = 0; q < nr; ++q) {
+          const v2d t = *reinterpret_cast<const v2d*>(p + (int64_t)q * ldt);
+          a0 = fma(t.x, zs[q], a0);
+          a1 = fma(t.y, zs[q], a1);
+        }
+      } else {
+        for (int q = 0; q < nr; ++q) {
+          const v2d t = *reinterpret_cast<const v2d*>(p + (int64_t)q * ldt);
+          a0 = (k <= i0 + q) ? fma(t.x, zs[q], a0) : a0;
+          a1 = (k + 1 <= i0 + q) ? fma(t.y, zs[q], a1) : a1;
+        }
+      }
+      v2d o;
+      o.x = a0;
+      o.y = a1;
+      *reinterpret_cast<v2d*>(slot + k) = o;
+    }
+    __syncthreads();
+  }
+}
+
+__global__ __launch_bounds__(1024) void gpp_mll_alpha_finish(const double* __restrict__ L, int64_t ld, int64_t N,
+                                                             const double* __restrict__ z, double* __restrict__ out3,
+                                                             const double* __restrict__ part, int64_t C,
+                                                             double* __restrict__ alpha) {
+  __shared__ double sq[16], sl[16];
+  if (blockIdx.x == 0) {
+    mll_scalars_block(L, ld, N, z, out3, sq, sl);
+    return;
+  }
+  const int64_t k = ((int64_t)blockIdx.x - 1) * 1024 + threadIdx.x;
+  if (k >= N) return;
+  double s = 0.0;
+#pragma unroll 8
+  for (int64_t c = k / MA_ROWS; c < C; ++c) s += part[ma_slot(c) + k];
+  alpha[k] = s;
 }
 
 __global__ __launch_bounds__(256) void gpp_loo_rows(const double* __restrict__ Linv, int64_t ldi, int64_t N,
@@ -777,6 +859,21 @@
   return hipGetLastError();
 }
 
+size_t gpp_mll_alpha_ws_bytes(int64_t N) {
+  const int64_t C = (N + MA_ROWS - 1) / MA_ROWS;
+  return (size_t)ma_slot(C) * sizeof(double);
+}
+
+hipError_t gpp_launch_mll_reduce_alpha(hipStream_t s, const double* L, int64_t ld, const double* T, int64_t ldt, int64_t N,
+                                       const double* r, double* z, double* out3, double* alpha, void* ws, size_t ws_bytes) {
+  if (N > 0 && (!ws || ws_bytes < gpp_mll_alpha_ws_bytes(N))) return hipErrorInvalidValue;
+  const int64_t C = (N + MA_ROWS - 1) / MA_ROWS;
+  double* part = reinterpret_cast<double*>(ws);
+  if (N > 0) hipLaunchKernelGGL(gpp_mll_alpha_rows, dim3((unsigned)((C + 1) / 2)), dim3(1024), 0, s, T, ldt, N, r, z, part, C);
+  hipLaunchKernelGGL(gpp_mll_alpha_finish, dim3((unsigned)(1 + (N + 1023) / 1024)), dim3(1024), 0, s, L, ld, N, z, out3, part, C, alpha);
+  return hipGetLastError();
+}
+
 size_t gpp_trmv_t_ws_bytes(int64_t N) { return (size_t)TRT_CHUNKS * (size_t)N * sizeof(double); }
 
 hipError_t gpp_launch_trmv_lower_cols(hipStream_t s, const double* T, int64_t ldt, int64_t N, const double* x, double* y,
diff --git a/gp-plus_amd/linalg.py b/gp-plus_amd/linalg.py
--- a/gp-plus_amd/linalg.py
+++ b/gp-plus_amd/linalg.py
@@ -194,12 +194,22 @@
             g_Ud = torch.empty(N, dU, dtype=torch.float64, device=dev) if need_U else None
         ops, grads = (Ud, wd, sd, grp, S), (dU if need_U else 0, g_w, g_s, g_t, g_Ud)
 
+        want_alpha = need_grad or fn.value_needs_alpha
+        lower = fn.lower_only
+
         def rest():
             with _stage("trtri"):
-                gctx.trtri(ws.A, ws.Li, ws.Ki)
+                (gctx.trtri_lower if lower else gctx.trtri)(ws.A, ws.Li, ws.Ki)
+            if lower and want_alpha:
+                with _stage("mll_reduce"):
+                    gctx.mll_reduce_alpha(ws.A, ws.Li, ws.r, ws.z, ws.out3, ws.alpha)
+                with _stage("alpha"):
+                    pass
+                fn.tail(gctx, ws, need_grad, ops, grads, kind, d_split)
+                return
             with _stage("mll_reduce"):
                 gctx.mll_reduce(ws.A, ws.Li, ws.r, ws.z, ws.out3)
-            if need_grad or fn.value_needs_alpha:
+            if want_alpha:
                 with _stage("alpha"):
                     gctx.alpha(ws.Li, ws.z, ws.alpha)
             fn.tail(gctx, ws, need_grad, ops, grads, kind, d_split)
@@ -212,7 +222,7 @@
 
 class ExactMLLFunction(torch.autograd.Function):
 
-    capturable, value_needs_alpha = True, False
+    capturable, value_needs_alpha, lower_only = True, False, True
 
     @staticmethod
     def forward(ctx, U, w, sf2, tau, mean, y, grp, kind, d_split, dU, slot):
@@ -257,7 +267,7 @@
 
 class ExactLOOFunction(torch.autograd.Function):
 
-    capturable, value_needs_alpha = False, True
+    capturable, value_needs_alpha, lower_only = False, True, False
 
     @staticmethod
     def forward(ctx, U, w, sf2, tau, mean, y, grp, kind, d_split, dU, slot):
@@ -305,7 +315,7 @@
 
 class _CVEvaluation:
 
-    capturable, value_needs_alpha, what = False, True, "the cross-validation objective"
+    capturable, value_needs_alpha, lower_only, what = False, True, False, "the cross-validation objective"
 
     def __init__(self, folds):
         self.folds, self.terms, self.infos = folds, None, None
diff --git a/include/gpp.h b/include/gpp.h
--- a/include/gpp.h
+++ b/include/gpp.h
@@ -75,6 +75,10 @@
                        int64_t ldi, double* T, int64_t ldt, int32_t* info_dev);
 
 int gpp_trtri(gpp_handle_t h, const double* U, int64_t N, int64_t ld, double* Linv, int64_t ldi, double* T, int64_t ldt);
+
+int gpp_trtri_lower(gpp_handle_t h, const double* U, int64_t N, int64_t ld, double* Linv, int64_t ldi, double* T, int64_t ldt);
+
+int gpp_trtri_complete_mirror(gpp_handle_t h, double* Linv, int64_t N, int64_t ldi);
 
 int gpp_lauum(gpp_handle_t h, const double* Linv, int64_t N, int64_t ldi, double* Kinv, int64_t ldk);
 
@@ -157,6 +161,9 @@
 int gpp_mll_reduce(gpp_handle_t h, const double* U, int64_t ld, const double* Linv, int64_t ldi, int64_t N,
                    const double* r, double* z, double* out3);
 
+int gpp_mll_reduce_alpha(gpp_handle_t h, const double* U, int64_t ld, const double* Linv, int64_t ldi, int64_t N, const double* r,
+                         double* z, double* out3, double* alpha);
+
 int gpp_alpha(gpp_handle_t h, const double* Linv, int64_t ldi, int64_t N, const double* z, double* alpha);
 
 int gpp_grad_reduce(gpp_handle_t h, const double* U, int64_t N, int D, const double* w, const double* sf2,
```

After: 7.711 evals/s. No clear change (-0.0%).
